# DerekGloudemans/3D-playground

Hardware: AMD Instinct MI355X
Metric: training images/sec at 1920x1080, ResNet-50 3D-RetinaNet (higher is better)
Workload: dtype f32; 1 GPU; resnet50 directional 3D-RetinaNet, 1920x1080 synthetic frames, batch 8 per GPU, 10 GT boxes/image, fp32, fwd+loss+bwd+clip+Adam (BASELINE configs[1]); global_batch=8, parallelism=dp1

## Files before the change

### 3d-playground_amd/csrc/conv_wino.hip

```cpp
#include "common.h"
#include "mfma_split.h"

__device__ __forceinline__ float4 f4(float s) { return make_float4(s, s, s, s); }
typedef float nt_f4 __attribute__((ext_vector_type(4)));
__device__ __forceinline__ float4 ld_stream(const float *p) {
    const nt_f4 v = __builtin_nontemporal_load(reinterpret_cast<const nt_f4 *>(p));
    return make_float4(v.x, v.y, v.z, v.w);
}
__device__ __forceinline__ void st_stream(float *p, float4 v) { *reinterpret_cast<float4 *>(p) = v; }
__device__ __forceinline__ float4 operator+(float4 a, float4 b) { return make_float4(a.x + b.x, a.y + b.y, a.z + b.z, a.w + b.w); }
__device__ __forceinline__ float4 operator-(float4 a, float4 b) { return make_float4(a.x - b.x, a.y - b.y, a.z - b.z, a.w - b.w); }
__device__ __forceinline__ float4 operator*(float s, float4 a) { return make_float4(s * a.x, s * a.y, s * a.z, s * a.w); }

__device__ __forceinline__ void bt6(const float4 d[6], float4 o[6]) {
    o[0] = 4.f * d[0] - 5.f * d[2] + d[4];
    o[1] = d[3] + d[4] - 4.f * (d[1] + d[2]);
    o[2] = 4.f * (d[1] - d[2]) - d[3] + d[4];
    o[3] = 2.f * (d[3] - d[1]) - d[2] + d[4];
    o[4] = 2.f * (d[1] - d[3]) - d[2] + d[4];
    o[5] = 4.f * d[1] - 5.f * d[3] + d[5];
}
__device__ __forceinline__ void at6(const float4 m[6], float4 o[4]) {
    const float4 s12 = m[1] + m[2], d12 = m[1] - m[2], s34 = m[3] + m[4], d34 = m[3] - m[4];
    o[0] = m[0] + s12 + s34;
// ... 16 lines not shown
    unsigned *amax[RN_MAX_GROUP];
};

#define WINO_GAIN_BT 7
#define WINO_GAIN_A 8
__device__ __forceinline__ void wino_tensor_word(const WinoTable &g, unsigned *tensor_amax, int gain) {
    if (tensor_amax == nullptr || blockIdx.x != 0 || threadIdx.x >= 64) return;
    int e = 0;
#pragma unroll
    for (int i = 0; i < RN_MAX_GROUP; ++i)
        if (i < g.n && g.amax[i] != nullptr) { const int ei = rn_amax_exp_all(g.amax[i], g.p[i].N); e = ei > e ? ei : e; }
    if (threadIdx.x == 0) atomicMax(tensor_amax, rn_amax_word_of_exp(e, gain));
}
__device__ __forceinline__ int wino_locate(const WinoTable &g, int64_t gt, int64_t &local) {
    int q = 0;
#pragma unroll
    for (int i = 0; i < RN_MAX_GROUP - 1; ++i) q += (i + 1 < g.n && gt >= g.tile_end[i]) ? 1 : 0;
    int64_t first = 0;
#pragma unroll
    for (int i = 1; i < RN_MAX_GROUP; ++i)
        if (q == i) first = g.tile_end[i - 1];
    local = gt - first;
    return q;
}

#define WINO_SELECT(q, g, pr, EXTRA)                          \
    WinoProblem pr = g.p[0];                                   \
    _Pragma("unroll") for (int i_ = 1; i_ < RN_MAX_GROUP; ++i_) \
        if (q == i_) { pr = g.p[i_]; EXTRA }

__global__ __launch_bounds__(256) void wino_in_kernel(const WinoTable g, float *__restrict__ V, int C, int64_t t0, int64_t Tpad,
                                                      unsigned *__restrict__ row_amax, unsigned *__restrict__ tensor_amax) {
    wino_tensor_word(g, tensor_amax, WINO_GAIN_BT);
    const int cq = C >> 2;
    const int64_t id = (int64_t)xcd_remap(blockIdx.x, gridDim.x) * 256 + threadIdx.x;
    const int64_t gt_raw = id / cq, t_last = g.tile_end[g.n - 1];
    const int64_t gt = gt_raw < t_last ? gt_raw : t_last - 1;
    const int c4 = (int)(id - gt_raw * cq) * 4;
    int64_t tile;
    const int q = wino_locate(g, gt, tile);
    const float *x = g.src[0];
    const unsigned *xw = g.amax[0];
    WINO_SELECT(q, g, pr, x = g.src[i_]; xw = g.amax[i_];)
    const int H = pr.H, W = pr.W, TW = pr.TW;
    const int n = (int)(tile / (pr.TH * TW));
    const int r = (int)(tile - (int64_t)n * pr.TH * TW);
    const int th = r / TW, tw = r - th * TW;
    const int h0 = 4 * th - 1, w0 = 4 * tw - 1;
    const float *xb = x + (int64_t)n * H * W * C + c4;
    if (row_amax != nullptr) {
        const int e_img = rn_amax_exp_lanes(xw != nullptr ? reinterpret_cast<const unsigned char *>(xw) + (int64_t)n * RN_AMAX_BYTES : nullptr);
        if (gt_raw < t_last && c4 == 0) row_amax[t0 + gt] = rn_amax_word_of_exp(e_img, WINO_GAIN_BT);
    }
    if (gt_raw >= t_last) return;
    float4 t[6][6];
#pragma unroll
    for (int j = 0; j < 6; ++j) {
        float4 d[6], o[6];
        const int w = w0 + j;
#pragma unroll
        for (int i = 0; i < 6; ++i) {
            const int h = h0 + i;
#ifdef RN_WINO_ABL
            const bool ok = (unsigned)h < (unsigned)H && (unsigned)w < (unsigned)W && i >= 1 && i <= 4 && j >= 1 && j <= 4;
#else
            const bool ok = (unsigned)h < (unsigned)H && (unsigned)w < (unsigned)W;
#endif
            d[i] = ok ? *reinterpret_cast<const float4 *>(xb + ((int64_t)h * W + w) * C) : f4(0.f);
        }
        bt6(d, o);
#pragma unroll
        for (int i = 0; i < 6; ++i) t[i][j] = o[i];
    }
    float *vb = V + (t0 + gt) * C + c4;
#pragma unroll
    for (int i = 0; i < 6; ++i) {
        float4 o[6];
        bt6(t[i], o);
#pragma unroll
        for (int j = 0; j < 6; ++j) st_stream(vb + (int64_t)(i * 6 + j) * Tpad * C, o[j]);
    }
}

template <bool PBITS, bool PADD, bool FLAGS = false>
__global__ __launch_bounds__(256, 2) void wino_out_kernel(const WinoTable g, const float *__restrict__ M, int Cout, int64_t t0,
                                                       int64_t Tpad, const float *__restrict__ scale,
                                                       const float *__restrict__ shift, int mask_mode, int act, int64_t y_bs,
                                                       const unsigned char *__restrict__ fin = nullptr,
                                                       unsigned char *__restrict__ fout = nullptr) {
    const int cq = Cout >> 2;
    const int64_t id = (int64_t)blockIdx.x * 256 + threadIdx.x;
    const int64_t gt = id / cq;
    float am = 0.f;
    unsigned *yam = nullptr;
    int n_img = 0;
    bool live = false;
    do {
    if (gt >= g.tile_end[g.n - 1]) break;
    live = true;
    const int c4 = (int)(id - gt * cq) * 4;
    int64_t tile;
    const int q = wino_locate(g, gt, tile);
    float *y = g.dst[0];
    const float *add = g.add[0], *mask = g.mask[0];
    unsigned *sign = g.sign[0];
    yam = g.amax[0];
    WINO_SELECT(q, g, pr, y = g.dst[i_]; add = g.add[i_]; mask = g.mask[i_]; sign = g.sign[i_]; yam = g.amax[i_];)
    n_img = (int)(tile / (pr.TH * pr.TW));
    const bool mbits = (mask_mode & RN_MASK_BITS) != 0;
    mask_mode &= 3;
    const int H = pr.H, W = pr.W, TW = pr.TW;
    const int n = (int)(tile / (pr.TH * TW));
    const int r = (int)(tile - (int64_t)n * pr.TH * TW);
    const int th = r / TW, tw = r - th * TW;
    const float *mb = M + (t0 + gt) * Cout + c4;
    float4 t[4][6];
    bool active = true;
    if constexpr (FLAGS) active = fin == nullptr || fin[t0 + gt] != 0;
    if (active) {
#pragma unroll
        for (int j = 0; j < 6; ++j) {
            float4 m[6], o[4];
#pragma unroll
            for (int i = 0; i < 6; ++i) m[i] = ld_stream(mb + (int64_t)(i * 6 + j) * Tpad * Cout);
            at6(m, o);
#pragma unroll
            for (int i = 0; i < 4; ++i) t[i][j] = o[i];
        }
    } else {
#pragma unroll
        for (int j = 0; j < 6; ++j)
#pragma unroll
            for (int i = 0; i < 4; ++i) t[i][j] = f4(0.f);
    }
    unsigned wake = 0u;
    float4 sc = f4(1.f), sh = f4(0.f);
    if (scale) sc = *reinterpret_cast<const float4 *>(scale + c4);
    if (shift) sh = *reinterpret_cast<const float4 *>(shift + c4);
    const int64_t ybs = y_bs ? y_bs : (int64_t)H * W * Cout;
#pragma unroll
    for (int i = 0; i < 4; ++i) {
        float4 o[4];
        at6(t[i], o);
        const int oh = 4 * th + i;
        if (oh >= H) break;
        unsigned mkw[4];
        float4 adv[4];
        if constexpr (PBITS || PADD) {
#pragma unroll
            for (int j = 0; j < 4; ++j) {
                const int owc = 4 * tw + j < W ? 4 * tw + j : W - 1;
                const int64_t off = (((int64_t)n * H + oh) * W + owc) * Cout + c4;
                if constexpr (PBITS) mkw[j] = reinterpret_cast<const unsigned *>(mask)[off >> 5] >> ((unsigned)off & 28u);
                if constexpr (PADD) adv[j] = *reinterpret_cast<const float4 *>(add + off);
            }
        }
#pragma unroll
        for (int j = 0; j < 4; ++j) {
            const int ow = 4 * tw + j;
            if (ow >= W) break;
            const int64_t off = (((int64_t)n * H + oh) * W + ow) * Cout + c4;
            const int64_t yoff = (int64_t)n * ybs + ((int64_t)oh * W + ow) * Cout + c4;
            float v[4] = {sc.x * o[j].x + sh.x, sc.y * o[j].y + sh.y, sc.z * o[j].z + sh.z, sc.w * o[j].w + sh.w};
            float mk[4] = {1.f, 1.f, 1.f, 1.f}, ad[4] = {0.f, 0.f, 0.f, 0.f};
            if constexpr (PBITS) {
                const unsigned nb = mkw[j];
                mk[0] = (nb & 1u) ? 1.f : 0.f; mk[1] = (nb & 2u) ? 1.f : 0.f; mk[2] = (nb & 4u) ? 1.f : 0.f; mk[3] = (nb & 8u) ? 1.f : 0.f;
            } else if (mask_mode != 0) { const float4 q4 = rn_mask_load4(mask, off, mbits); mk[0] = q4.x; mk[1] = q4.y; mk[2] = q4.z; mk[3] = q4.w; }
            if constexpr (PADD) { const float4 q4 = adv[j]; ad[0] = q4.x; ad[1] = q4.y; ad[2] = q4.z; ad[3] = q4.w; }
            else if (add) { const float4 q4 = *reinterpret_cast<const float4 *>(add + off); ad[0] = q4.x; ad[1] = q4.y; ad[2] = q4.z; ad[3] = q4.w; }
#pragma unroll
            for (int k = 0; k < 4; ++k) {
                float u = v[k];
                if (mask_mode == 1) u = mk[k] > 0.f ? u : 0.f;
                u += ad[k];
                if (act == 1) u = fmaxf(u, 0.f);
                else if (act == 2) u = 1.0f / (1.0f + expf(-u));
                if (mask_mode == 2) u = mk[k] > 0.f ? u : 0.f;
                v[k] = u;
            }
            *reinterpret_cast<float4 *>(y + yoff) = make_float4(v[0], v[1], v[2], v[3]);
            if (sign != nullptr) rn_sign_store(sign, off, v[0], v[1], v[2], v[3]);
            am = fmaxf(fmaxf(am, fmaxf(fabsf(v[0]), fabsf(v[1]))), fmaxf(fabsf(v[2]), fabsf(v[3])));
// ... 292 lines not shown
    int64_t end = 0;
    for (int i = 0; i < RN_MAX_GROUP; ++i) {
        const int k = i < g->n ? i : g->n - 1;
        if (g->N[k] <= 0 || g->H[k] <= 0 || g->W[k] <= 0) return RN_EINVAL;
        t.p[i].N = g->N[k]; t.p[i].H = g->H[k]; t.p[i].W = g->W[k];
        t.p[i].TH = (g->H[k] + 3) / 4; t.p[i].TW = (g->W[k] + 3) / 4;
        if (i < g->n) end += (int64_t)g->N[k] * t.p[i].TH * t.p[i].TW;
        t.tile_end[i] = end;
        t.src[i] = g->src[k]; t.dst[i] = g->dst[k]; t.add[i] = g->add[k]; t.mask[i] = g->mask[k];
        t.sign[i] = reinterpret_cast<unsigned *>(g->sign[k]);
        t.amax[i] = reinterpret_cast<unsigned *>(g->amax[k]);
    }
    return RN_OK;
}

extern "C" int rn_wino_input_group(const rn_wino_group *g, float *V, int C, int64_t tile_offset, int64_t Tpad, int dy_form,
                                   void *row_amax, void *tensor_amax, void *stream) {
    WinoTable t;
    const int rc = wino_table(g, t);
    if (rc) return rc;
    if (C <= 0 || (C & 3) || tile_offset < 0 || tile_offset + t.tile_end[t.n - 1] > Tpad) return RN_EINVAL;
    for (int i = 0; i < t.n; ++i)
        if (!t.src[i]) return RN_EINVAL;
    const dim3 grid(rn_blocks(t.tile_end[t.n - 1] * (C >> 2), 256));
    if (dy_form && row_amax != nullptr) return RN_EINVAL;
    if (dy_form) hipLaunchKernelGGL(wino_dy_kernel, grid, dim3(256), 0, (hipStream_t)stream, t, V, C, tile_offset, Tpad,
                                    reinterpret_cast<unsigned *>(tensor_amax));
    else hipLaunchKernelGGL(wino_in_kernel, grid, dim3(256), 0, (hipStream_t)stream, t, V, C, tile_offset, Tpad,
                            reinterpret_cast<unsigned *>(row_amax), reinterpret_cast<unsigned *>(tensor_amax));
    RN_LAUNCH_CHECK();
    return RN_OK;
}

extern "C" int rn_wino_input_both_group_flags(const rn_wino_group *g, float *V, float *Z, int C, int64_t tile_offset, int64_t Tpad,
                                              void *v_row_amax, void *z_tensor_amax, const void *flags, void *stream) {
    WinoTable t;
    const int rc = wino_table(g, t);
    if (rc) return rc;
    if (!V || !Z || C <= 0 || (C & 3) || tile_offset < 0 || tile_offset + t.tile_end[t.n - 1] > Tpad) return RN_EINVAL;
    if (flags != nullptr && (((uintptr_t)flags & 15) || (Tpad & 15))) return RN_EINVAL;
    for (int i = 0; i < t.n; ++i)
        if (!t.src[i]) return RN_EINVAL;
    const dim3 grid(rn_blocks(t.tile_end[t.n - 1] * (C >> 2), 256));
    if (flags != nullptr)
        hipLaunchKernelGGL(wino_in_both_kernel<true>, grid, dim3(256), 0, (hipStream_t)stream, t, V, Z, C, tile_offset, Tpad,
                           reinterpret_cast<unsigned *>(v_row_amax), reinterpret_cast<unsigned *>(z_tensor_amax),
                           reinterpret_cast<const unsigned char *>(flags));
    else
        hipLaunchKernelGGL(wino_in_both_kernel<false>, grid, dim3(256), 0, (hipStream_t)stream, t, V, Z, C, tile_offset, Tpad,
                           reinterpret_cast<unsigned *>(v_row_amax), reinterpret_cast<unsigned *>(z_tensor_amax),
                           (const unsigned char *)nullptr);
    RN_LAUNCH_CHECK();
    return RN_OK;
}
extern "C" int rn_tile_lists(const void *flags, int64_t Tpad, void *counts, void *tiles, void *units, void *blocks, void *stream) {
    if (!flags || !counts || !tiles || !units || !blocks || Tpad <= 0 || (Tpad & 255) || Tpad > 256 * 128) return RN_EINVAL;
    if (((uintptr_t)flags & 15) || (((uintptr_t)counts | (uintptr_t)tiles | (uintptr_t)units | (uintptr_t)blocks) & 3)) return RN_EINVAL;
    hipLaunchKernelGGL(tile_lists_kernel, dim3(1), dim3(256), 0, (hipStream_t)stream, reinterpret_cast<const unsigned char *>(flags), (int)Tpad,
                       reinterpret_cast<int *>(counts), reinterpret_cast<int *>(tiles), reinterpret_cast<int *>(units),
                       reinterpret_cast<int *>(blocks));
    RN_LAUNCH_CHECK();
    return RN_OK;
}

extern "C" int rn_wino_input_both_group_lists(const rn_wino_group *g, float *V, float *Z, int C, int64_t tile_offset, int64_t Tpad,
                                              void *v_row_amax, void *z_tensor_amax, const void *flags, const void *units,
                                              const void *n_units, void *stream) {
    WinoTable t;
    const int rc = wino_table(g, t);
    if (rc) return rc;
    if (!V || !Z || C <= 0 || (C & 3) || tile_offset < 0 || tile_offset + t.tile_end[t.n - 1] > Tpad) return RN_EINVAL;
    if (!flags || !units || !n_units || ((uintptr_t)flags & 15) || ((uintptr_t)units & 3) || (Tpad & 15)) return RN_EINVAL;
    for (int i = 0; i < t.n; ++i)
        if (!t.src[i]) return RN_EINVAL;
    const dim3 gl(rn_blocks(t.tile_end[t.n - 1] * (C >> 2), 256));
    hipLaunchKernelGGL((wino_in_both_kernel<true, true>), gl, dim3(256), 0, (hipStream_t)stream, t, V, Z, C, tile_offset, Tpad,
                       reinterpret_cast<unsigned *>(v_row_amax), reinterpret_cast<unsigned *>(z_tensor_amax),
                       reinterpret_cast<const unsigned char *>(flags), reinterpret_cast<const int *>(units),
                       reinterpret_cast<const int *>(n_units));
    RN_LAUNCH_CHECK();
    return RN_OK;
}

extern "C" int rn_wino_input_both_group(const rn_wino_group *g, float *V, float *Z, int C, int64_t tile_offset, int64_t Tpad,
                                        void *v_row_amax, void *z_tensor_amax, void *stream) {
    return rn_wino_input_both_group_flags(g, V, Z, C, tile_offset, Tpad, v_row_amax, z_tensor_amax, nullptr, stream);
}

extern "C" int rn_wino_output_group_flags(const rn_wino_group *g, const float *M, int Cout, int64_t tile_offset, int64_t Tpad,
                                          const float *scale, const float *shift, int mask_mode, int act, int64_t y_batch_stride,
                                          const void *flags_in, void *flags_out, void *stream) {
    WinoTable t;
    const int rc = wino_table(g, t);
    if (rc) return rc;
    if (Cout <= 0 || (Cout & 3) || tile_offset < 0 || tile_offset + t.tile_end[t.n - 1] > Tpad) return RN_EINVAL;
    if (mask_mode < 0 || (mask_mode & ~(3 | RN_MASK_BITS)) || (mask_mode & 3) == 3 || mask_mode == RN_MASK_BITS) return RN_EINVAL;
    if (act < 0 || act > 2 || y_batch_stride < 0 || (y_batch_stride & 3)) return RN_EINVAL;
    for (int i = 0; i < t.n; ++i) {
        if (!t.dst[i] || (mask_mode != 0) != (t.mask[i] != nullptr)) return RN_EINVAL;
        if (((mask_mode & RN_MASK_BITS) || t.sign[i]) && (Cout & 31)) return RN_EINVAL;
        if (y_batch_stride && y_batch_stride < (int64_t)t.p[i].H * t.p[i].W * Cout) return RN_EINVAL;
    }
    const bool pbits = (mask_mode & RN_MASK_BITS) != 0;
    bool padd = true;
    for (int i = 0; i < t.n; ++i) padd = padd && t.add[i] != nullptr;
    const dim3 grid(rn_blocks(t.tile_end[t.n - 1] * (Cout >> 2), 256));
    const unsigned char *fin = reinterpret_cast<const unsigned char *>(flags_in);
    unsigned char *fout = reinterpret_cast<unsigned char *>(flags_out);
#define RN_WINO_OUT(B, A, F) hipLaunchKernelGGL((wino_out_kernel<B, A, F>), grid, dim3(256), 0, (hipStream_t)stream, t, M, Cout, tile_offset, Tpad, \
                                                scale, shift, mask_mode, act, y_batch_stride, fin, fout)
    if (fin != nullptr || fout != nullptr) {
        if (pbits && padd) RN_WINO_OUT(true, true, true);
        else if (pbits) RN_WINO_OUT(true, false, true);
        else if (padd) RN_WINO_OUT(false, true, true);
        else RN_WINO_OUT(false, false, true);
    } else if (pbits && padd) RN_WINO_OUT(true, true, false);
    else if (pbits) RN_WINO_OUT(true, false, false);
    else if (padd) RN_WINO_OUT(false, true, false);
    else RN_WINO_OUT(false, false, false);
#undef RN_WINO_OUT
    RN_LAUNCH_CHECK();
    return RN_OK;
}
extern "C" int rn_wino_output_group(const rn_wino_group *g, const float *M, int Cout, int64_t tile_offset, int64_t Tpad,
                                    const float *scale, const float *shift, int mask_mode, int act, int64_t y_batch_stride,
                                    void *stream) {
    return rn_wino_output_group_flags(g, M, Cout, tile_offset, Tpad, scale, shift, mask_mode, act, y_batch_stride, nullptr, nullptr, stream);
}

static rn_wino_group wino_single(const float *src, float *dst, const float *add, const float *mask, int N, int H, int W) {
    rn_wino_group g = {};
    g.n = 1; g.N[0] = N; g.H[0] = H; g.W[0] = W; g.src[0] = src; g.dst[0] = dst; g.add[0] = add; g.mask[0] = mask;
    return g;
}
extern "C" int rn_wino_input(const float *x, float *V, int N, int H, int W, int C, int64_t tile_offset, int64_t Tpad,
                             void *stream) {
    const rn_wino_group g = wino_single(x, nullptr, nullptr, nullptr, N, H, W);
    return rn_wino_input_group(&g, V, C, tile_offset, Tpad, 0, nullptr, nullptr, stream);
}
extern "C" int rn_wino_dy(const float *dy, float *Z, int N, int H, int W, int C, int64_t tile_offset, int64_t Tpad, void *stream) {
    const rn_wino_group g = wino_single(dy, nullptr, nullptr, nullptr, N, H, W);
    return rn_wino_input_group(&g, Z, C, tile_offset, Tpad, 1, nullptr, nullptr, stream);
}
extern "C" int rn_wino_output(const float *M, float *y, int N, int H, int W, int Cout, int64_t tile_offset, int64_t Tpad,
                              const float *scale, const float *shift, const float *add, const float *mask, int mask_mode,
                              int act, int64_t y_batch_stride, void *stream) {
    const rn_wino_group g = wino_single(nullptr, y, add, mask, N, H, W);
    return rn_wino_output_group(&g, M, Cout, tile_offset, Tpad, scale, shift, mask_mode, act, y_batch_stride, stream);
}

extern "C" int rn_wino_weights(const float *w, float *U, int Cout, int Cin, int mode, const float *scale, void *stream) {
    if (Cout <= 0 || Cin <= 0 || mode < 0 || mode > 1) return RN_EINVAL;
    const int rows = mode == 0 ? Cout : Cin;
    const int Kpad = ((mode == 0 ? Cin : Cout) + 31) / 32 * 32;
    hipLaunchKernelGGL(wino_weight_kernel, dim3(rn_blocks((int64_t)rows * Kpad, 256)), dim3(256), 0, (hipStream_t)stream, w, U,
                       Cout, Cin, mode, scale, rows, Kpad);
    RN_LAUNCH_CHECK();
    return RN_OK;
}

extern "C" int rn_wino_dw(const float *dU, float *dw, int Cout, int Cin, void *stream) {
    if (Cout <= 0 || Cin <= 0) return RN_EINVAL;
    const int Ku = (Cin + 31) / 32 * 32, Kpad = (9 * Cin + 31) / 32 * 32;
    hipLaunchKernelGGL(wino_dw_kernel, dim3(rn_blocks((int64_t)Cout * Cin, 256)), dim3(256), 0, (hipStream_t)stream, dU, dw, Cout,
                       Cin, Ku, Kpad);
    RN_LAUNCH_CHECK();
    return RN_OK;
}
```

### 3d-playground_amd/csrc/focal_loss.hip

```cpp
#include <math.h>
#include <stdlib.h>

#include "common.h"

#ifndef FOCAL_NTHR
#define FOCAL_NTHR 256
#endif
#define NTHR FOCAL_NTHR
#define APT 4
#define TILE (NTHR * APT)
#define NWAVES (NTHR / 64)
#define UAPT 2
#define UNIT (64 * UAPT)
#define QCAP 256
#ifndef RN_FOCAL_WAVES_PER_SIMD
#define RN_FOCAL_WAVES_PER_SIMD 4
#endif
#define RN_FOCAL_WAVES_NOTE 4
#define RN_FOCAL_RESIDENT 768

static inline int focal_resident() {
    static const int v = [] { const char *e = getenv("RN_FOCAL_RESIDENT"); const int x = e ? atoi(e) : 0; return x >= 8 ? x : RN_FOCAL_RESIDENT; }();
    return v;
}
// ... 734 lines not shown
    const int units = (int)((A + UNIT - 1) / UNIT);
    const FocalWs ws = focal_ws(workspace, B);
    const dim3 grid((unsigned)(B * G)), block(NTHR);
    const float4 *anc = reinterpret_cast<const float4 *>(anchors);
    const int cq = C == 4 ? 1 : (C == 8 ? 2 : 0);
    const size_t raw_bytes = (size_t)(N > 0 ? N : 1) * (directional ? 27 : 5) * sizeof(float);
#define RN_FOCAL_FWD(DIR_, CQ_)                                                                                        \
    hipLaunchKernelGGL((focal_kernel<DIR_, false, CQ_>), grid, block, raw_bytes, s, cls, reg, anc, ann, A, C, N,        \
                       ws.partials, ws.stats, (float *)nullptr, (float *)nullptr, G, units, ws.counter, ws.terms, losses, \
                       (const float *)nullptr)
    if (directional) {
        if (cq == 2) RN_FOCAL_FWD(true, 2); else if (cq == 1) RN_FOCAL_FWD(true, 1); else RN_FOCAL_FWD(true, 0);
    } else {
        if (cq == 2) RN_FOCAL_FWD(false, 2); else if (cq == 1) RN_FOCAL_FWD(false, 1); else RN_FOCAL_FWD(false, 0);
    }
#undef RN_FOCAL_FWD
    RN_LAUNCH_CHECK();
    return RN_OK;
}

extern "C" int rn_focal_loss_bwd(const float *cls, const float *reg, const float *anchors, const float *ann, int B,
                                 int64_t A, int C, int N, int directional, const void *workspace,
                                 const float *grad_losses, float *dcls, float *dreg, void *stream) {
    const int rc = check_args(B, A, C, N);
    if (rc) return rc;
    hipStream_t s = (hipStream_t)stream;
    const int G = focal_groups(B, A);
    const int units = (int)((A + UNIT - 1) / UNIT);
    const FocalWs ws = focal_ws(const_cast<void *>(workspace), B);
    const dim3 grid((unsigned)(B * G)), block(NTHR);
    const float4 *anc = reinterpret_cast<const float4 *>(anchors);
    const int cq = C == 4 ? 1 : (C == 8 ? 2 : 0);
    const size_t raw_bytes = (size_t)(N > 0 ? N : 1) * (directional ? 27 : 5) * sizeof(float);
#define RN_FOCAL_BWD(DIR_, CQ_)                                                                                      \
    hipLaunchKernelGGL((focal_kernel<DIR_, true, CQ_>), grid, block, raw_bytes, s, cls, reg, anc, ann, A, C, N,       \
                       (float *)nullptr, ws.stats, dcls, dreg, G, units, (unsigned *)nullptr, (double *)nullptr,      \
                       (float *)nullptr, grad_losses)
    if (directional) {
        if (cq == 2) RN_FOCAL_BWD(true, 2); else if (cq == 1) RN_FOCAL_BWD(true, 1); else RN_FOCAL_BWD(true, 0);
    } else {
        if (cq == 2) RN_FOCAL_BWD(false, 2); else if (cq == 1) RN_FOCAL_BWD(false, 1); else RN_FOCAL_BWD(false, 0);
    }
#undef RN_FOCAL_BWD
    RN_LAUNCH_CHECK();
    return RN_OK;
}

template <bool DIR>
__global__ __launch_bounds__(NTHR) void assign_kernel(const float4 *__restrict__ anchors, const float *__restrict__ ann,
                                                      int64_t A, int N, float *__restrict__ iou_max,
                                                      int32_t *__restrict__ argmax, int32_t *__restrict__ state) {
    constexpr int COLS = DIR ? 27 : 5;
    __shared__ LabelLds L;
    const int j = blockIdx.y;
    load_labels<DIR>(ann + (int64_t)j * N * COLS, N, L);
    const int64_t ai = (int64_t)blockIdx.x * NTHR + threadIdx.x;
    if (ai >= A) return;
    float best = 0.f; int arg = -1; int st = 0;
    if (L.count > 0) {
        match_anchor(anchors[ai], L, best, arg);
        st = -1;
        if (best < 0.4f) st = 0;
        if (best >= 0.5f) st = 1;
    }
    iou_max[(int64_t)j * A + ai] = best;
    argmax[(int64_t)j * A + ai] = arg;
    state[(int64_t)j * A + ai] = st;
}

extern "C" int rn_assign(const float *anchors, const float *ann, int B, int64_t A, int N, int directional,
                         float *iou_max, int32_t *argmax, int32_t *state, void *stream) {
    const int rc = check_args(B, A, 1, N);
    if (rc) return rc;
    const dim3 grid((unsigned)((A + NTHR - 1) / NTHR), B), block(NTHR);
    const float4 *anc = reinterpret_cast<const float4 *>(anchors);
    if (directional)
        hipLaunchKernelGGL(assign_kernel<true>, grid, block, 0, (hipStream_t)stream, anc, ann, A, N, iou_max, argmax, state);
    else
        hipLaunchKernelGGL(assign_kernel<false>, grid, block, 0, (hipStream_t)stream, anc, ann, A, N, iou_max, argmax, state);
    RN_LAUNCH_CHECK();
    return RN_OK;
}

__global__ void pairwise_iou_kernel(const float4 *__restrict__ a, const float4 *__restrict__ b, float *__restrict__ out,
                                    int64_t A, int N) {
    const int64_t i = (int64_t)blockIdx.x * 256 + threadIdx.x;
    if (i >= A * N) return;
    const int64_t ai = i / N;
    const int n = (int)(i - ai * N);
    const float4 p = a[ai], q = b[n];
    const float area_b = (q.z - q.x) * (q.w - q.y);
    float iw = fminf(p.z, q.z) - fmaxf(p.x, q.x);
    float ih = fminf(p.w, q.w) - fmaxf(p.y, q.y);
    iw = fmaxf(iw, 0.f);
    ih = fmaxf(ih, 0.f);
    float ua = ((p.z - p.x) * (p.w - p.y) + area_b) - iw * ih;
    ua = fmaxf(ua, 1e-8f);
    out[i] = (iw * ih) / ua;
}

extern "C" int rn_pairwise_iou(const float *a, const float *b, float *iou, int64_t A, int N, void *stream) {
    if (A <= 0 || N <= 0) return RN_EINVAL;
    hipLaunchKernelGGL(pairwise_iou_kernel, dim3(rn_blocks(A * N, 256)), dim3(256), 0, (hipStream_t)stream,
                       reinterpret_cast<const float4 *>(a), reinterpret_cast<const float4 *>(b), iou, A, N);
    RN_LAUNCH_CHECK();
    return RN_OK;
}
```

### 3d-playground_amd/retinanet_mi355x/_hip.py

```python
import ctypes
import os

import torch

_HERE = os.path.dirname(os.path.abspath(__file__))
LIB_PATH = os.environ.get("RN_LIB_PATH") or os.path.join(_HERE, "lib", "libretinanet_mi355x.so")
_lib = None

c_i32, c_i64, c_f32, c_f64, c_vp = ctypes.c_int, ctypes.c_int64, ctypes.c_float, ctypes.c_double, ctypes.c_void_p

SIGNATURES = {
    "rn_version": (ctypes.c_char_p, []),
    "rn_check_device": (c_i32, []),
    "rn_get_fp32_mfma": (c_i32, []),
    "rn_set_fp32_mfma": (c_i32, [c_i32]),
    "rn_get_option": (c_i32, [c_i32]),
    "rn_set_option": (c_i32, [c_i32, c_i32]),
    "rn_fp32_split_min_k": (c_i32, []),
    "rn_split_weights": (c_i32, [c_vp, c_vp, c_i64, c_i32, c_vp]),
    "rn_split_weights_f16": (c_i32, [c_vp, c_vp, c_vp, c_i64, c_i32, c_vp]),
    "rn_amax": (c_i32, [c_vp, c_i64, c_i32, c_vp, c_vp]),
    "rn_stream_capture_id": (c_i32, [c_vp, ctypes.POINTER(ctypes.c_ulonglong)]),
    "rn_anchor_count": (c_i64, [c_i32, c_i32]),
    "rn_anchor_base_boxes": (None, [c_vp]),
    "rn_anchors_fwd": (c_i32, [c_vp, c_i32, c_i32, c_vp]),
    "rn_pairwise_iou": (c_i32, [c_vp, c_vp, c_vp, c_i64, c_i32, c_vp]),
    "rn_focal_workspace_bytes": (c_i64, [c_i32, c_i64]),
    "rn_focal_workspace_zero_bytes": (c_i64, [c_i32]),
    "rn_focal_loss_fwd": (c_i32, [c_vp, c_vp, c_vp, c_vp, c_i32, c_i64, c_i32, c_i32, c_i32, c_vp, c_vp, c_vp]),
    "rn_focal_loss_bwd": (c_i32, [c_vp, c_vp, c_vp, c_vp, c_i32, c_i64, c_i32, c_i32, c_i32, c_vp, c_vp, c_vp, c_vp, c_vp]),
    "rn_assign": (c_i32, [c_vp, c_vp, c_i32, c_i64, c_i32, c_i32, c_vp, c_vp, c_vp, c_vp]),
    "rn_decode_dir": (c_i32, [c_vp, c_vp, c_vp, c_i32, c_i64, c_vp]),
    "rn_decode_dir_select": (c_i32, [c_vp, c_vp, c_i64, c_vp, c_i64, c_vp, c_vp, c_i32, c_vp, c_vp, c_vp, c_vp]),
    "rn_decode_2d": (c_i32, [c_vp, c_vp, c_vp, c_i32, c_i64, c_i32, c_f32, c_f32, c_vp]),
    "rn_clip_boxes": (c_i32, [c_vp, c_i64, c_f32, c_f32, c_vp]),
    "rn_post_workspace_bytes": (c_i64, [c_i64, c_i64]),
    "rn_rowmax": (c_i32, [c_vp, c_i64, c_i32, c_vp, c_vp, c_vp]),
    "rn_threshold_select": (c_i32, [c_vp, c_i64, c_i64, c_f64, c_i32, c_f64, c_vp, c_vp, c_vp, c_vp]),
    "rn_nms": (c_i32, [c_vp, c_i64, c_i32, c_vp, c_i64, c_vp, c_vp, c_vp, c_i32, c_f32, c_vp, c_vp, c_vp, c_vp]),
    "rn_state_to_space": (c_i32, [c_vp, c_vp, c_i64, c_vp]),
    "rn_space_to_state": (c_i32, [c_vp, c_vp, c_i64, c_vp]),
    "rn_state_to_im": (c_i32, [c_vp, c_vp, c_vp, c_vp, c_vp, c_i64, c_vp]),
    "rn_space_to_im": (c_i32, [c_vp, c_vp, c_vp, c_vp, c_vp, c_i64, c_vp]),
    "rn_im_to_space": (c_i32, [c_vp, c_vp, c_vp, c_vp, c_vp, c_vp, c_i64, c_vp]),
    "rn_im_to_state": (c_i32, [c_vp, c_vp, c_vp, c_vp, c_vp, c_vp, c_i64, c_vp]),
    "rn_parse_workspace_bytes": (c_i64, [c_i64]),
    "rn_parse_detections": (c_i32, [c_vp, c_vp, c_vp, c_vp, c_i64, c_vp, c_vp, c_vp, c_vp, c_i32, c_vp, c_f32, c_f32, c_f32,
                                    c_i32, c_i32, c_vp, c_vp, c_vp, c_vp, c_vp, c_vp, c_vp]),
    "rn_md_iou": (c_i32, [c_vp, c_vp, c_vp, c_i64, c_vp]),
    "rn_crop_boxes": (c_i32, [c_vp, c_vp, c_i32, c_f64, c_vp, c_vp, c_vp]),
    "rn_roi_align": (c_i32, [c_vp, c_i32, c_i32, c_i32, c_i32, c_vp, c_i32, c_i32, c_i32, c_vp, c_i32, c_vp]),
    "rn_crop_select": (c_i32, [c_vp] * 9 + [c_i32] * 4 + [c_f64, c_i32, c_f32, c_vp, c_vp, c_vp, c_vp]),
    "rn_kf_view": (c_i32, [c_vp, c_vp, c_vp, c_vp, c_i32, c_i32, c_vp, c_i32, c_vp]),
    "rn_kf_predict": (c_i32, [c_vp, c_vp, c_vp, c_vp, c_vp, c_vp, c_vp, c_i32, c_f64, c_i32, c_vp]),
    "rn_kf_update": (c_i32, [c_vp, c_vp, c_vp, c_vp, c_vp, c_vp, c_vp, c_i32, c_vp]),
    "rn_track_cost": (c_i32, [c_vp, c_i64, c_vp, c_i64, c_i64, c_i64, c_vp, c_vp]),
    "rn_lsap_workspace_bytes": (c_i64, [c_i64, c_i64]),
    "rn_linear_sum_assignment": (c_i32, [c_vp, c_i64, c_i64, c_f64, c_vp, c_vp, c_vp, c_vp, c_vp]),
    "rn_ts_bias_workspace_bytes": (c_i64, [c_i64, c_i64]),
    "rn_estimate_ts_bias": (c_i32, [c_vp, c_i64, c_vp, c_i64, c_vp, c_vp, c_i64, c_i64, c_vp, c_vp, c_i32, c_f64, c_f64, c_f32,
                                    c_vp, c_i64, c_vp, c_vp, c_vp, c_vp]),
    "rn_track_crop_prior": (c_i32, [c_vp] * 7 + [c_i32, c_vp, c_vp, c_vp, c_i32, c_vp]),
    "rn_fit_nearest": (c_i32, [c_vp, c_vp, c_vp, c_i64, c_i64, c_vp, c_vp, c_vp, c_vp]),
    "rn_residual_moments": (c_i32, [c_vp, c_i64, c_i32, c_vp, c_i32, c_vp, c_vp, c_vp, c_vp]),
    "rn_eval_select": (c_i32, [c_vp, c_vp, c_vp, c_i64, c_i64, c_i64, c_f32, c_i32, c_i32, c_i64, c_i32, c_vp, c_i64, c_vp, c_vp, c_vp]),
    "rn_eval_match": (c_i32, [c_vp, c_i64, c_vp, c_i64, c_i32, c_vp, c_vp, c_i64, c_f64, c_vp, c_vp, c_vp, c_vp]),
    "rn_eval_ap_workspace_bytes": (c_i64, [c_i64]),
    "rn_eval_ap": (c_i32, [c_vp, c_i64, c_vp, c_vp, c_vp, c_i32, c_vp, c_vp, c_vp, c_vp]),
    "rn_eval_corners": (c_i32, [c_vp, c_i64, c_i64, c_i32, c_i64, c_vp, c_vp, c_i64, c_vp, c_vp]),
    "rn_eval_cuboid_overlap": (c_i32, [c_vp, c_i64, c_vp, c_i64, c_i32, c_vp, c_vp, c_vp, c_i64, c_i32, c_vp, c_vp, c_vp]),
    "rn_eval_cuboid_assign": (c_i32, [c_vp, c_i64, c_vp, c_i64, c_i32, c_vp, c_i64, c_vp, c_vp, c_vp, c_i32, c_vp, c_vp, c_vp,
                                      c_vp, c_vp]),
    "rn_eval_cuboid_errors": (c_i32, [c_vp, c_i64, c_vp, c_i64, c_i32, c_vp, c_vp, c_vp, c_i64, c_vp, c_vp, c_vp, c_vp, c_vp,
                                      c_vp]),
    "rn_frame_ingest": (c_i32, [c_vp, c_i32, c_i32, c_i32, c_i32] + [c_f32] * 6 + [c_i32, c_vp, c_vp]),
    "rn_frame_ingest_half": (c_i32, [c_vp, c_i32, c_i32, c_i32, c_i32] + [c_f32] * 6 + [c_i32, c_vp, c_vp, c_vp]),
    "rn_parse_frame_timestamps": (c_i32, [c_vp, c_i32, c_i32, c_i32, c_i64, c_i64, c_i32, c_vp, c_i32] + [c_vp] * 9),
    "rn_augment_workspace_bytes": (c_i64, [c_i32, c_i32, c_i32]),
    "rn_augment_frames": (c_i32, [c_vp, c_i32, c_i32, c_i32, c_vp, c_vp, c_vp, c_vp, ctypes.c_uint64] + [c_f32] * 6 + [c_vp, c_vp, c_vp]),
    "rn_augment_crops_workspace_bytes": (c_i64, [c_i32, c_i32, c_i32]),
    "rn_augment_crops": (c_i32, [c_vp, c_i32, c_i32, c_i32, c_vp, c_vp, c_vp, c_vp, c_vp, c_i32, c_i32, c_i32, c_vp, c_vp, ctypes.c_uint64]
                         + [c_f32] * 6 + [c_vp, c_vp, c_vp]),
    "rn_mot_prepare": (c_i32, [c_vp, c_vp, c_vp, c_i64, c_vp, c_i64] + [c_vp] * 7),
    "rn_mot_iou": (c_i32, [c_vp] * 5 + [c_i64, c_i64, c_vp, c_vp]),
    "rn_mot_assign": (c_i32, [c_vp] * 5 + [c_i64] * 4 + [c_vp] * 5),
    "rn_mot_frame_metrics": (c_i32, [c_vp] * 5 + [c_i64, c_i64, c_vp, c_vp, c_vp, c_f64] + [c_vp] * 19),
    "rn_mot_workspace_bytes": (c_i64, [c_i64, c_i64]),
    "rn_mot_reduce": (c_i32, [c_i64, c_i64] + [c_vp] * 16 + [c_i64, c_i64, c_vp, c_vp, c_vp]),
    "rn_mot_assoc_workspace_bytes": (c_i64, [c_i64, c_i64]),
    "rn_mot_id_counts": (c_i32, [c_vp] * 5 + [c_i64] * 6 + [c_vp, c_vp, c_i64, c_i64, c_f64] + [c_vp] * 5),
    "rn_mot_id_assign": (c_i32, [c_vp, c_i64, c_i64, c_vp, c_vp, c_vp, c_vp]),
    "rn_mot_hota_align": (c_i32, [c_vp] * 5 + [c_i64] * 6 + [c_vp] * 5 + [c_i64] * 3 + [c_vp] * 5),
    "rn_mot_hota_assign": (c_i32, [c_vp] * 5 + [c_i64] * 6 + [c_vp, c_vp, c_i64, c_i64] + [c_vp] * 11),
    "rn_mot_hota_reduce": (c_i32, [c_vp] * 4 + [c_i64] * 6 + [c_vp] * 9 + [c_i64, c_i64, c_vp, c_vp, c_vp]),
    "rn_vanishing_points": (c_i32, [c_vp, c_i64, c_vp, c_i64, c_vp, c_vp, c_vp, c_vp]),
    "rn_hg_reproj_error": (c_i32, [c_vp, c_vp, c_vp, c_vp, c_vp, c_i64, c_i64, c_vp, c_vp]),
    "rn_hg_scale_z": (c_i32, [c_vp, c_vp, c_vp, c_vp, c_i64, c_f64, c_f64, c_i32, c_vp, c_vp, c_vp, c_vp]),
    "rn_fit_homography": (c_i32, [c_vp, c_vp, c_i64, c_vp, c_i64, c_i32, c_vp, c_vp, c_vp]),
    "rn_reinterp_mate": (c_i32, [c_vp, c_vp, c_i64, c_i64, c_vp, c_vp, c_vp]),
    "rn_reinterp_offsets": (c_i32, [c_vp, c_vp, c_i64, c_i64, c_vp, c_i64] + [c_vp] * 5),
    "rn_reinterp_rows": (c_i32, [c_vp] * 7 + [c_i64] * 4 + [c_vp] * 5),
    "rn_track_rows": (c_i32, [c_vp] * 5 + [c_i64, c_i64] + [c_vp] * 7),
    "rn_render_edges": (c_i32, [c_vp, c_vp, c_i64, c_i32, c_i32, c_vp, c_i32, c_i32, c_i32, c_vp]),
    "rn_render_rects": (c_i32, [c_vp, c_i64, c_vp, c_i64, c_vp, c_i32, c_i32, c_i32, c_vp]),
    "rn_render_text": (c_i32, [c_vp, c_i64, c_vp, c_i64, c_vp, c_vp, c_i64, c_vp, c_i32, c_i32, c_i32, c_vp]),
    "rn_render_compose": (c_i32, [c_vp] + [c_f32] * 6 + [c_vp, c_i32, c_vp, c_i32, c_i32, c_i32, c_i32, c_vp]),
    "rn_replay_boxes": (c_i32, [c_vp, c_i64, c_vp, c_vp, c_vp, c_i32, c_vp, c_vp, c_vp, c_vp, c_vp]),
    "rn_replay_compose": (c_i32, [c_vp, c_i32, c_vp, c_vp] + [c_i32] * 6 + [c_vp]),
    "rn_frame_absdiff": (c_i32, [c_vp, c_vp] + [c_i32] * 6 + [c_vp, c_vp, c_vp]),
    "rn_running_frame": (c_i32, [c_vp, c_vp, c_i64, c_i32, c_vp]),
    "rn_label_pair_samples": (c_i32, [c_vp, c_vp, c_i64, c_i32, c_i64, c_i32, c_i32, c_i32, c_vp, c_vp, c_vp, c_vp]),
    "rn_label_outliers": (c_i32, [c_vp, c_vp, c_vp, c_i64, c_i64, c_i64, c_i64, c_vp, c_vp, c_vp]),
    "rn_label_interpolate_workspace_bytes": (c_i64, [c_i64, c_i64]),
    "rn_label_interpolate": (c_i32, [c_vp] * 4 + [c_i64] * 3 + [c_i32, c_i64] + [c_vp] * 7),
    "rn_label_rebase": (c_i32, [c_vp, c_vp, c_i64] + [c_vp] * 4 + [c_i32, c_vp, c_i32, c_i32] + [c_vp] * 5),
    "rn_label_offset_y": (c_i32, [c_vp] * 4 + [c_i64, c_i32, c_vp, c_vp]),
    "rn_label_crop_windows": (c_i32, [c_vp, c_vp, c_i64, c_vp, c_vp, c_i32, c_f32, c_f32, c_f32] + [c_vp] * 6),
    "rn_label_best_anchor": (c_i32, [c_vp, c_vp, c_vp, c_i64, c_i32, c_i32, c_f32] + [c_vp] * 5),
    "rn_label_fit_box2d": (c_i32, [c_vp] * 5 + [c_i64, c_vp, c_vp, c_i32, c_vp, c_i32, c_i32] + [c_vp] * 5),
    "rn_spline_fit_workspace_bytes": (c_i64, [c_i64, c_i32]),
    "rn_label_box_weights": (c_i32, [c_vp, c_vp, c_i64, c_vp, c_vp, c_i32, c_vp, c_vp, c_vp]),
    "rn_spline_fit": (c_i32, [c_vp, c_i64, c_vp, c_i64, c_vp, c_vp, c_vp, c_i64, c_vp, c_i64, c_i32] + [c_vp] * 7),
    "rn_spline_select": (c_i32, [c_vp, c_i64] + [c_vp] * 4 + [c_i64, c_i64, c_i64, c_i32] + [c_vp] * 4 + [c_i32] + [c_vp] * 7),
    "rn_spline_eval": (c_i32, [c_vp, c_vp, c_vp, c_i64, c_i32, c_vp, c_vp, c_i64, c_vp, c_vp]),
    "rn_label_ts_shift": (c_i32, [c_vp, c_vp, c_vp, c_i64, c_i32, c_vp, c_vp, c_vp, c_i64, c_i64, c_vp, c_vp, c_vp, c_i32, c_i32,
                                  c_i32] + [c_vp] * 5),
    "rn_label_series_workspace_bytes": (c_i64, [c_i64]),
    "rn_label_series": (c_i32, [c_vp, c_vp, c_i64, c_i32, c_i64, c_i32, c_f64, c_f64, c_i32] + [c_vp] * 8),
    "rn_label_group_rmse": (c_i32, [c_vp, c_vp, c_i64, c_i64] + [c_vp] * 5),
    "rn_stitch_endpoints": (c_i32, [c_vp, c_vp, c_vp, c_i64, c_i64, c_i32, c_vp, c_vp, c_vp]),
    "rn_stitch_costs": (c_i32, [c_vp, c_i64] + [c_f64] * 7 + [c_vp, c_vp]),
    "rn_stitch_candidates": (c_i32, [c_vp, c_i64] + [c_f64] * 7 + [c_vp] * 4),
    "rn_stitch_compact": (c_i32, [c_vp, c_i64] + [c_f64] * 7 + [c_vp, c_vp, c_i64, c_vp, c_vp, c_vp]),
    "rn_stitch_assign_workspace_bytes": (c_i64, [c_i64]),
    "rn_stitch_assign": (c_i32, [c_vp, c_i64] + [c_f64] * 7 + [c_vp, c_vp, c_vp, c_i64] + [c_vp] * 6),
    "rn_stitch_chains": (c_i32, [c_vp, c_vp, c_i64] + [c_vp] * 6),
    "rn_stitch_fill_count": (c_i32, [c_vp, c_vp, c_i64, c_f64] + [c_vp] * 4),
    "rn_stitch_fill_rows": (c_i32, [c_vp, c_vp, c_vp, c_i64, c_i64, c_f64] + [c_vp] * 6),
    "rn_smooth_filter": (c_i32, [c_vp] * 5 + [c_f64, c_f64, c_i64, c_i64] + [c_vp] * 5),
    "rn_smooth_rts": (c_i32, [c_vp] * 5 + [c_f64, c_i64, c_i64] + [c_vp] * 4),
    "rn_traffic_lanes": (c_i32, [c_vp] * 4 + [c_i32, c_vp, c_i32, c_i64, c_i64] + [c_vp] * 4),
    "rn_traffic_cells": (c_i32, [c_vp] * 4 + [c_i32, c_vp, c_i32, c_i64, c_i64, c_f64, c_f64, c_i64, c_f64, c_f64, c_i64, c_f64] + [c_vp] * 6),
    "rn_traffic_leaders": (c_i32, [c_vp] * 6 + [c_i64] * 4 + [c_vp] * 8),
}

class ConvDesc(ctypes.Structure):
    _fields_ = [("N", c_i32), ("Hi", c_i32), ("Wi", c_i32), ("Cin", c_i32),
                ("Ho", c_i32), ("Wo", c_i32), ("Cout", c_i32),
                ("kh", c_i32), ("kw", c_i32),
                ("a", c_i32), ("b", c_i32), ("p", c_i32), ("p_w", c_i32), ("div_shift", c_i32),
                ("act", c_i32), ("add_mode", c_i32), ("Ha", c_i32), ("Wa", c_i32),
                ("mask_mode", c_i32), ("in_relu", c_i32),
                ("os", c_i32), ("oo_h", c_i32), ("oo_w", c_i32), ("Hy", c_i32), ("Wy", c_i32),
                ("add2_mode", c_i32), ("Ha2", c_i32), ("Wa2", c_i32), ("add2_batch_stride", c_i64),
                ("x_batch_stride", c_i64), ("y_batch_stride", c_i64), ("add_batch_stride", c_i64),
                ("w_batch_stride", c_i64), ("w_format", c_i32), ("sign_out", c_vp),
                ("x_amax", c_vp), ("y_amax", c_vp), ("w_unscale", c_vp), ("x_amax_img_stride", c_i32), ("x_amax_row_stride", c_i32),
                ("row_active", c_vp), ("row_list", c_vp), ("row_list_n", c_vp), ("row_list_grid", c_i32)]


RN_MAX_GROUP = 5


class ConvGroup(ctypes.Structure):
    _fields_ = [("n", c_i32), ("tile_end", c_i32 * RN_MAX_GROUP), ("d", ConvDesc * RN_MAX_GROUP),
                ("x", c_vp * RN_MAX_GROUP), ("y", c_vp * RN_MAX_GROUP), ("add", c_vp * RN_MAX_GROUP),
                ("mask", c_vp * RN_MAX_GROUP)]


class PrepJob(ctypes.Structure):
    _fields_ = [("kind", c_i32)] + [(n, c_i32) for n in ("Cout", "Cin", "kh", "kw", "kw_pad", "c_pad", "mode", "r0", "nr", "s0",
                                                          "ns", "rows", "Kpad")] + \
               [("eps", c_f32), ("src", c_vp), ("dst", c_vp), ("scale", c_vp), ("gamma", c_vp), ("beta", c_vp), ("mean", c_vp),
                ("var", c_vp), ("bn_scale", c_vp), ("bn_shift", c_vp), ("bn_rstd", c_vp)]


class UnpackJob(ctypes.Structure):
    _fields_ = [("dw", c_vp), ("w_packed", c_vp), ("dweight", c_vp)] + \
               [(n, c_i32) for n in ("Cout", "Cin", "kh", "kw", "kw_pad", "c_pad", "Kpad")] + \
               [("scale", c_vp), ("mean", c_vp), ("rstd", c_vp), ("colsum", c_vp), ("dgamma", c_vp), ("dbeta", c_vp)]


class WinoGroup(ctypes.Structure):
    _fields_ = [("n", c_i32), ("N", c_i32 * RN_MAX_GROUP), ("H", c_i32 * RN_MAX_GROUP), ("W", c_i32 * RN_MAX_GROUP),
                ("src", c_vp * RN_MAX_GROUP), ("dst", c_vp * RN_MAX_GROUP), ("add", c_vp * RN_MAX_GROUP),
                ("mask", c_vp * RN_MAX_GROUP), ("sign", c_vp * RN_MAX_GROUP), ("amax", c_vp * RN_MAX_GROUP)]


SIGNATURES.update({
    "rn_unpack_batched": (c_i32, [c_vp, c_vp, c_i32, c_vp]),
    "rn_prep_batched": (c_i32, [c_vp, c_vp, c_i32, c_vp]),
    "rn_wino_input_group": (c_i32, [ctypes.POINTER(WinoGroup), c_vp, c_i32, c_i64, c_i64, c_i32, c_vp, c_vp, c_vp]),
    "rn_wino_input_both_group": (c_i32, [ctypes.POINTER(WinoGroup), c_vp, c_vp, c_i32, c_i64, c_i64, c_vp, c_vp, c_vp]),
    "rn_wino_input_both_group_flags": (c_i32, [ctypes.POINTER(WinoGroup), c_vp, c_vp, c_i32, c_i64, c_i64, c_vp, c_vp, c_vp, c_vp]),
    "rn_tile_lists": (c_i32, [c_vp, c_i64, c_vp, c_vp, c_vp, c_vp, c_vp]),
    "rn_wino_input_both_group_lists": (c_i32, [ctypes.POINTER(WinoGroup), c_vp, c_vp, c_i32, c_i64, c_i64, c_vp, c_vp, c_vp, c_vp, c_vp, c_vp]),
    "rn_wino_output_group_flags": (c_i32, [ctypes.POINTER(WinoGroup), c_vp, c_i32, c_i64, c_i64, c_vp, c_vp, c_i32, c_i32, c_i64, c_vp, c_vp, c_vp]),
    "rn_wino_output_group": (c_i32, [ctypes.POINTER(WinoGroup), c_vp, c_i32, c_i64, c_i64, c_vp, c_vp, c_i32, c_i32, c_i64, c_vp]),
    "rn_conv_igemm_grouped": (c_i32, [ctypes.POINTER(ConvGroup), c_vp, c_vp, c_vp, c_vp]),
    "rn_conv_igemm": (c_i32, [ctypes.POINTER(ConvDesc), c_vp, c_vp, c_vp, c_vp, c_vp, c_vp, c_vp, c_vp, c_vp]),
    "rn_conv_splitk_workspace_bytes": (c_i64, [ctypes.POINTER(ConvDesc)]),
    "rn_conv_igemm_wants_f16": (c_i32, [ctypes.POINTER(ConvDesc)]),
    "rn_conv_igemm_splitk": (c_i32, [ctypes.POINTER(ConvDesc)] + [c_vp] * 10),
    "rn_conv_wgrad": (c_i32, [c_vp, c_i32, c_vp, c_vp, c_vp] + [c_i32] * 12 + [c_vp]),
    "rn_pack_weights": (c_i32, [c_vp, c_vp] + [c_i32] * 7 + [c_vp] + [c_i32] * 4 + [c_vp]),
    "rn_unpack_wgrad": (c_i32, [c_vp, c_vp, c_vp] + [c_i32] * 6 + [c_vp] * 7),
    "rn_bn_fold": (c_i32, [c_vp, c_vp, c_vp, c_vp, c_f32, c_i32, c_vp, c_vp, c_vp, c_vp]),
    "rn_nchw_to_nhwc4": (c_i32, [c_vp, c_vp, c_i32, c_i32, c_i32, c_vp, c_vp]),
    "rn_maxpool_fwd": (c_i32, [c_vp, c_vp, c_vp] + [c_i32] * 6 + [c_vp]),
    "rn_maxpool_bwd": (c_i32, [c_vp, c_vp, c_vp, c_vp] + [c_i32] * 7 + [c_vp, c_vp]),
    "rn_colsum": (c_i32, [c_vp, c_i64, c_i32, c_i32, c_vp, c_i32, c_vp, c_vp]),
    "rn_colsum_workspace_bytes": (c_i64, [c_i64, c_i32]),
    "rn_upsample_add_bwd": (c_i32, [c_vp, c_vp] + [c_i32] * 6 + [c_vp, c_vp]),
    "rn_relu_mask": (c_i32, [c_vp, c_vp, c_i64, c_vp]),
    "rn_sigmoid_bwd_pad": (c_i32, [c_vp, c_vp, c_vp, c_i32, c_i64, c_i32, c_i32, c_i64, c_vp, c_vp]),
    "rn_sigmoid_bwd_pad_flags": (c_i32, [c_vp, c_vp, c_vp, c_i32, c_i32, c_i32, c_i32, c_i32, c_i64, c_vp, c_vp, c_vp]),
    "rn_add_inplace": (c_i32, [c_vp, c_vp, c_i64, c_i64, c_vp, c_vp]),
    "rn_wino_input": (c_i32, [c_vp, c_vp, c_i32, c_i32, c_i32, c_i32, c_i64, c_i64, c_vp]),
    "rn_wino_output": (c_i32, [c_vp, c_vp, c_i32, c_i32, c_i32, c_i32, c_i64, c_i64, c_vp, c_vp, c_vp, c_vp, c_i32, c_i32, c_i64, c_vp]),
    "rn_wino_weights": (c_i32, [c_vp, c_vp, c_i32, c_i32, c_i32, c_vp, c_vp]),
    "rn_wino_dy": (c_i32, [c_vp, c_vp, c_i32, c_i32, c_i32, c_i32, c_i64, c_i64, c_vp]),
    "rn_wino_dw": (c_i32, [c_vp, c_vp, c_i32, c_i32, c_vp]),
    "rn_conv_wgrad_batched": (c_i32, [c_vp, c_i32, c_vp, c_vp, c_vp, c_i32, c_i64, c_i64, c_i64, c_i32] + [c_i32] * 12 + [c_vp, c_i32, c_vp, c_i32, c_vp]),
    "rn_conv_wgrad_batched_det": (c_i32, [c_vp, c_i32, c_vp, c_vp, c_vp, c_i32, c_i64, c_i64, c_i64, c_i32] + [c_i32] * 12 + [c_vp, c_i32, c_vp, c_i32, c_vp, c_i64, c_vp]),
    "rn_conv_wgrad_batched_flags": (c_i32, [c_vp, c_i32, c_vp, c_vp, c_vp, c_i32, c_i64, c_i64, c_i64, c_i32] + [c_i32] * 12 + [c_vp, c_i32, c_vp, c_i32, c_vp, c_vp, c_i64, c_vp]),
    "rn_conv_wgrad_det_workspace_bytes": (c_i64, [c_i32, c_i32, c_i64] + [c_i32] * 9),
    "rn_conv_wgrad_plan": (c_i32, [c_i32, c_i32, c_i64, c_i64, c_i64, c_i32] + [c_i32] * 12 + [c_i32, c_i32, c_i32, c_vp]),
    "rn_conv_bwd_1x1": (c_i32, [c_vp] * 8 + [c_i32] + [c_vp] * 5 + [c_i32] * 6 + [c_vp]),
    "rn_f32_to_bf16": (c_i32, [c_vp, c_vp, c_i64, c_vp]),
    "rn_bf16_to_f32": (c_i32, [c_vp, c_vp, c_i64, c_vp]),
    "rn_conv_igemm_bf16": (c_i32, [ctypes.POINTER(ConvDesc), c_vp, c_vp, c_vp, c_i32, c_vp, c_vp, c_vp, c_vp, c_vp]),
    "rn_conv_igemm_bf16_grouped": (c_i32, [ctypes.POINTER(ConvGroup), c_vp, c_i32, c_vp, c_vp, c_vp]),
    "rn_conv_igemm_bf16_tile_rows": (c_i32, [ctypes.POINTER(ConvGroup), c_i32]),
    "rn_maxpool_fwd_fp8out": (c_i32, [c_vp, c_vp] + [c_i32] * 6 + [c_f32, c_vp]),
    "rn_conv_igemm_fp8_tile_rows": (c_i32, [ctypes.POINTER(ConvGroup), c_i32]),
    "rn_conv_igemm_fp8_tile": (c_i32, [ctypes.POINTER(ConvDesc), c_i32]),
    "rn_conv_igemm_bf16_tile": (c_i32, [ctypes.POINTER(ConvDesc), c_i32]),
    "rn_fp8_quantize": (c_i32, [c_vp, c_vp, c_i64, c_f32, c_vp]),
    "rn_fp8_dequantize": (c_i32, [c_vp, c_vp, c_i64, c_f32, c_vp]),
    "rn_fp8_to_bf16": (c_i32, [c_vp, c_vp, c_i64, c_f32, c_vp]),
    "rn_bf16_to_fp8": (c_i32, [c_vp, c_vp, c_i64, c_f32, c_vp]),
    "rn_fp8_quantize_rows": (c_i32, [c_vp, c_vp, c_vp, c_i64, c_i32, c_vp]),
    "rn_conv_igemm_fp8": (c_i32, [ctypes.POINTER(ConvDesc), c_vp, c_vp, c_vp, c_i32, c_vp, c_vp, c_vp, c_f32, c_f32, c_vp]),
    "rn_conv_igemm_fp8_grouped": (c_i32, [ctypes.POINTER(ConvGroup), c_vp, c_i32, c_vp, c_vp, c_f32, c_f32, c_vp]),
    "rn_conv_wgrad_bf16": (c_i32, [c_vp, c_i32, c_vp, c_vp, c_vp] + [c_i32] * 11 + [c_vp]),
    "rn_conv_wgrad_bf16_grouped": (c_i32, [c_i32, ctypes.POINTER(c_vp), c_i32, ctypes.POINTER(c_vp), c_vp, c_vp, c_i32,
                                           ctypes.POINTER(c_i32), ctypes.POINTER(c_i32)] + [c_i32] * 6 + [c_vp]),
    "rn_maxpool_fwd_bf16out": (c_i32, [c_vp, c_vp, c_vp] + [c_i32] * 6 + [c_vp]),
    "rn_maxpool_bwd_bf16in": (c_i32, [c_vp, c_vp, c_vp, c_vp] + [c_i32] * 7 + [c_vp]),
    "rn_upsample_add_bwd_bf16": (c_i32, [c_vp, c_vp] + [c_i32] * 6 + [c_vp]),
    "rn_sigmoid_bwd_pad_bf16": (c_i32, [c_vp, c_vp, c_vp, c_i32, c_i64, c_i32, c_i32, c_i64, c_vp]),
    "rn_relu_bf16": (c_i32, [c_vp, c_vp, c_i64, c_vp]),
    "rn_opt_workspace_bytes": (c_i64, [c_i32]),
    "rn_opt_clip_adam": (c_i32, [c_vp, c_vp, c_i32, c_f32, c_f32, c_f32, c_f32, c_f32, c_i32, c_i32, c_vp, c_vp, c_vp]),
    "rn_opt_clip_adam_dev": (c_i32, [c_vp, c_vp, c_i32, c_f32, c_f32, c_f32, c_f32, c_f32, c_vp, c_i32, c_vp, c_vp, c_vp]),
    "rn_opt_clip_adam_hp": (c_i32, [c_vp, c_vp, c_i32, c_vp, c_vp, c_i32, c_vp, c_vp, c_vp]),
})


RN_ERRORS = {10001: "RN_EINVAL (bad size / unsupported shape)",
             10002: "RN_ETOOMANY (more than RN_MAX_GT=256 label rows per image)"}


def load():
    global _lib
    if _lib is None:
        if not os.path.exists(LIB_PATH):
            raise RuntimeError(
                "libretinanet_mi355x.so is missing (%s): build it with `python -c 'import __graft_entry__ as g; "
                "g.build()'` or `make -C 3d-playground_amd/csrc`.  There is no CPU fallback." % LIB_PATH)
        lib = ctypes.CDLL(LIB_PATH)
        for name, (res, args) in SIGNATURES.items():
            fn = getattr(lib, name)
            fn.restype = res
            fn.argtypes = args
        _lib = lib
    return _lib

# ... 34 lines not shown
```

### 3d-playground_amd/retinanet_mi355x/conv.py

```python
import ctypes
import os

import torch

from . import _hip, prof

ConvDesc = _hip.ConvDesc

ACT_NONE, ACT_RELU, ACT_SIGMOID = 0, 1, 2


def kpad(kh, kw, c):
    return (kh * kw * c + 31) // 32 * 32


def out_size(n, k, stride, pad):
    return (n + 2 * pad - k) // stride + 1


def pack_weights(weight, mode=0, scale=None, kw_pad=None, c_pad=None, taps=None, presplit=True):
    lib = _hip.load()
    w = _hip.f32c(weight.detach())
    _hip.need_gpu(w, scale)
    cout, cin, kh, kw = w.shape
# ... 286 lines not shown
                return 1
            ws = torch.empty(nb, dtype=torch.uint8, device=dev)
        return lib.rn_conv_wgrad_batched_flags(dy_ptr, ldy, x_ptr, dw_ptr, cs_ptr, nbatch, dy_bs, x_bs, dw_bs, cs_batch, *geom, *am,
                                               flags.data_ptr(), _hip.ptr(ws), nb, _hip.stream())
    if not lib.rn_get_option(OPT_DETERMINISTIC):
        return lib.rn_conv_wgrad_batched(dy_ptr, ldy, x_ptr, dw_ptr, cs_ptr, nbatch, dy_bs, x_bs, dw_bs, cs_batch, *geom, *am, _hip.stream())
    N, Hi, Wi, Cin, Ho, Wo, Cout, kh, kw = geom[:9]
    nb = lib.rn_conv_wgrad_det_workspace_bytes(ldy, nbatch, dw_bs, N, Hi, Wi, Cin, Ho, Wo, Cout, kh, kw)
    if nb < 0:
        return 1
    ws = torch.empty(nb, dtype=torch.uint8, device=dev)
    return lib.rn_conv_wgrad_batched_det(dy_ptr, ldy, x_ptr, dw_ptr, cs_ptr, nbatch, dy_bs, x_bs, dw_bs, cs_batch, *geom, *am,
                                         ws.data_ptr(), nb, _hip.stream())


WGRAD_PLAN_FIELDS = ("shape", "tiles", "splits", "per_split", "xcd_map", "grid", "kernel", "arith")


def wgrad_plan(ldy, nbatch, dy_bs, x_bs, dw_bs, cs_batch, geom, have_amax=False, have_flags=False, det=None):
    out = (ctypes.c_int32 * 8)()
    det = get_option(OPT_DETERMINISTIC) if det is None else det
    rc = _hip.load().rn_conv_wgrad_plan(ldy, nbatch, dy_bs, x_bs, dw_bs, cs_batch, *geom, int(have_amax), int(have_flags), int(det), out)
    return dict(zip(WGRAD_PLAN_FIELDS, out)) if rc == 0 else None


def wino_weights(weight, mode=0, scale=None):
    lib = _hip.load()
    w = _hip.f32c(weight.detach())
    _hip.need_gpu(w, scale)
    cout, cin, kh, kw = w.shape
    assert kh == 3 and kw == 3
    rows, k = (cout, cin) if mode == 0 else (cin, cout)
    U = torch.empty((36, rows, (k + 31) // 32 * 32), dtype=torch.float32, device=w.device)
    _hip.check(lib.rn_wino_weights(w.data_ptr(), U.data_ptr(), cout, cin, mode, _hip.ptr(scale), _hip.stream()),
               "rn_wino_weights")
    return _maybe_split(U, rows=rows, cin=U.shape[2], taps=1)


_WINO_WS = {}
_WINO_ODD_PLANES = os.environ.get("RN_WINO_ODD_PLANES", "1") != "0"


def wino_tpad(T):
    n = (T + 255) // 256
    if _WINO_ODD_PLANES and n % 2 == 0:
        n += 1
    return n * 256


def _wino_group(xs, srcs=None, dsts=None, adds=None, masks=None, mask_bits=False, signs=None, amaxs=None):
    g = _hip.WinoGroup()
    g.n = len(xs)
    for i, x in enumerate(xs):
        g.N[i], g.H[i], g.W[i] = x.shape[0], x.shape[1], x.shape[2]
        g.src[i] = None if srcs is None else srcs[i].data_ptr()
        g.dst[i] = None if dsts is None else dsts[i].data_ptr()
        g.add[i] = None if adds is None or adds[i] is None else adds[i].data_ptr()
        if masks is None or masks[i] is None:
            g.mask[i] = None
        else:
            g.mask[i] = masks[i]._rn_sign.data_ptr() if mask_bits else masks[i].data_ptr()
        g.sign[i] = None if signs is None or signs[i] is None else signs[i].data_ptr()
        g.amax[i] = None if amaxs is None or amaxs[i] is None else amaxs[i].data_ptr()
    return g


def _wino_transform_in(xs, V, C, Tpad, dy_form, want_rows=False, want_tensor=False):
    lib = _hip.load()
    off = 0
    am = want_amax() and (want_rows or want_tensor)
    rows = torch.zeros(Tpad, dtype=torch.int32, device=V.device) if am and want_rows else None
    tword = amax_single(V.device) if am and want_tensor else None
    for k in range(0, len(xs), _hip.RN_MAX_GROUP):
        part = xs[k:k + _hip.RN_MAX_GROUP]
        t = sum(x.shape[0] * ((x.shape[1] + 3) // 4) * ((x.shape[2] + 3) // 4) for x in part)
        g = _wino_group(part, srcs=part, amaxs=[amax_words(x) for x in part] if am else None)
        nb = 4.0 * (sum(x.numel() for x in part) + 36 * t * C)
        _hip.check(prof.timed("wino_input", nb, lambda: lib.rn_wino_input_group(
            ctypes.byref(g), V.data_ptr(), C, off, Tpad, dy_form, _hip.ptr(rows), _hip.ptr(tword), _hip.stream())), "rn_wino_input_group")
        off += t
    return rows, tword


def _wino_workspace(device, floats_v, floats_m):
    key = (device, torch.cuda.current_stream(device).cuda_stream)
    ws = _WINO_WS.get(key)
    if ws is None or ws[0].numel() < floats_v or ws[1].numel() < floats_m:
        ws = (torch.empty(max(floats_v, ws[0].numel() if ws else 0), dtype=torch.float32, device=device),
              torch.empty(max(floats_m, ws[1].numel() if ws else 0), dtype=torch.float32, device=device))
        _WINO_WS[key] = ws
    return ws


def tile_flags(device, T):
    return torch.zeros(wino_tpad(T), dtype=torch.uint8, device=device)


class TileLists:
    __slots__ = ("flags", "buf", "counts", "tiles", "units", "blocks", "grid")

    def lengths(self):
        return tuple(int(v) for v in self.counts[:3].tolist())


def tile_lists_numel(Tpad):
    return 4 + Tpad + Tpad // 16 + Tpad // 128


def tile_lists(flags, Tpad=None, buf=None, grid=0):
    lib = _hip.load()
    Tpad = flags.numel() if Tpad is None else Tpad
    assert flags.dtype == torch.uint8 and flags.numel() >= Tpad and Tpad % 256 == 0
    n = tile_lists_numel(Tpad)
    if buf is None:
        buf = torch.empty(n, dtype=torch.int32, device=flags.device)
    assert buf.dtype == torch.int32 and buf.numel() >= n and buf.is_contiguous()
    tl = TileLists()
    tl.flags, tl.buf, tl.grid = flags, buf, int(grid)
    nb, nu = Tpad // 128, Tpad // 16
    tl.counts, tl.blocks, tl.units, tl.tiles = buf[:4], buf[4:4 + nb], buf[4 + nb:4 + nb + nu], buf[4 + nb + nu:n]
    _hip.check(lib.rn_tile_lists(flags.data_ptr(), Tpad, tl.counts.data_ptr(), tl.tiles.data_ptr(), tl.units.data_ptr(),
                                 tl.blocks.data_ptr(), _hip.stream()), "rn_tile_lists")
    return tl


def wino_flags_ok(T, C, cout):
    lib = _hip.load()
    return bool(get_fp32_mfma() != "native" and lib.rn_get_option(OPT_WGRAD_ONCE) and C > 64 and cout > 64 and T < 32000)


def wino_conv_group(xs, U, outs=None, scale=None, shift=None, act=ACT_NONE, adds=None, masks=None, mask_mode=2,
                    flops=0.0, keep_v=False, y_batch_stride=0, V_in=None, V_ready=None, sign=False, flags_out=None):
    lib = _hip.load()
    dev = xs[0].device
    C = xs[0].shape[3]
    cout = U.shape[1]
    tiles = [x.shape[0] * ((x.shape[1] + 3) // 4) * ((x.shape[2] + 3) // 4) for x in xs]
    T = sum(tiles)
    Tpad = wino_tpad(T)
    V, M = _wino_workspace(dev, 0 if keep_v else 36 * Tpad * C, 36 * Tpad * cout)
    shapes = tuple(tuple(x.shape) for x in xs)
    reuse = keep_v and V_in is not None and V_in[1] == shapes and V_in[0].numel() == 36 * Tpad * C
    ready = not keep_v and isinstance(V_ready, tuple) and V_ready[1] == shapes and V_ready[0].numel() >= 36 * Tpad * C
    if ready:
        V, reuse = V_ready[0], True
    elif reuse:
        V = V_in[0]
    elif keep_v:
        V = torch.empty(36 * Tpad * C, dtype=torch.float32, device=dev)
    assert all(x.is_contiguous() for x in xs)
    v_am = (None, None)
    if reuse:
        src = V_ready if ready else V_in
        v_am = src[2] if len(src) > 2 and src[2] is not None else (None, None)
    else:
        v_am = _wino_transform_in(xs, V, C, Tpad, 0, want_rows=True, want_tensor=keep_v)
    flags = V_ready[3] if ready and len(V_ready) > 3 else None
    lists = V_ready[4] if ready and len(V_ready) > 4 else None
    if flags_out is not None:
        assert flags_out.dtype == torch.uint8 and flags_out.numel() >= Tpad and len(xs) <= _hip.RN_MAX_GROUP
    Vv = V[:36 * Tpad * C].view(36, 1, Tpad, C)
    Mv = M[:36 * Tpad * cout].view(36, 1, Tpad, cout)
    Uv = _carry_split(U, U.view(36 * cout, U.shape[2]))
    if want_amax() and v_am[0] is None:
        Uv = U.view(36 * cout, U.shape[2])
    conv_igemm(Vv, Uv, Mv, (1, Tpad, cout, 1, 1, 1, 1, 0, 0), flops=2.0 * 36 * T * cout * C, w_batch_stride=cout * U.shape[2],
               x_amax=v_am[0], x_amax_rows=True, row_active=flags, row_list=lists)
    if outs is None:
        outs = [torch.empty((x.shape[0], x.shape[1], x.shape[2], cout), dtype=torch.float32, device=dev) for x in xs]
    off = 0
    for k in range(0, len(xs), _hip.RN_MAX_GROUP):
        sl = slice(k, k + _hip.RN_MAX_GROUP)
        part, t = xs[sl], sum(tiles[sl])
        pa = None if adds is None else adds[sl]
        pm = None if masks is None else masks[sl]
        has_mask = pm is not None and pm[0] is not None
        mbits = has_mask and BITMASKS and all(getattr(m, "_rn_sign", None) is not None for m in pm)
        for o in outs[sl]:
            amax_drop(o)
        signs = [_sign_words(o, sign and not y_batch_stride) for o in outs[sl]]
        yams = [amax_slot(dev, o.shape[0]) for o in outs[sl]] if want_amax() and not y_batch_stride else None
        g = _wino_group(part, dsts=outs[sl], adds=pa, masks=pm, mask_bits=mbits, signs=signs, amaxs=yams)
        nops = 1 + (pa is not None and pa[0] is not None) + (1.0 / 32 if mbits else 1.0) * has_mask + (1.0 / 32 if signs[0] is not None else 0.0)
        nb = 4.0 * (36 * t * cout + nops * sum(x.shape[0] * x.shape[1] * x.shape[2] for x in part) * cout)
        mm = (mask_mode | (MASK_BITS if mbits else 0)) if has_mask else 0
        if flags is not None or flags_out is not None:
            _hip.check(prof.timed("wino_output", nb, lambda: lib.rn_wino_output_group_flags(
                ctypes.byref(g), M.data_ptr(), cout, off, Tpad, _hip.ptr(scale), _hip.ptr(shift), mm,
                act, y_batch_stride, _hip.ptr(flags), _hip.ptr(flags_out), _hip.stream())), "rn_wino_output_group_flags")
        else:
            _hip.check(prof.timed("wino_output", nb, lambda: lib.rn_wino_output_group(
                ctypes.byref(g), M.data_ptr(), cout, off, Tpad, _hip.ptr(scale), _hip.ptr(shift), mm,
                act, y_batch_stride, _hip.stream())), "rn_wino_output_group")
        if yams is not None:
            for o, w_ in zip(outs[sl], yams):
                amax_attach(o, w_)
        off += t
    return (outs, (V, tuple(tuple(x.shape) for x in xs), v_am)) if keep_v else outs


_WINO_Z = {}
SIDE_HELD = {}


def side_release(side=None):
    if side is None:
        SIDE_HELD.clear()
    else:
        SIDE_HELD.pop(side.cuda_stream, None)


def _wino_z_buffer(device, floats):
    cur = torch.cuda.current_stream(device)
    st = _WINO_Z.setdefault((device, cur.cuda_stream), {"bufs": [None, None], "ev": [None, None], "i": 0})
    k = st["i"]
    st["i"] ^= 1
    if st["bufs"][k] is None or st["bufs"][k].numel() < floats:
        st["bufs"][k] = torch.empty(floats, dtype=torch.float32, device=device)
    if st["ev"][k] is not None:
        cur.wait_event(st["ev"][k])
    return st, k


def wino_wgrad_group(gs, xs, dw, colsum, flops=0.0, V=None, dU=None, fuse_dgrad_input=False, side=None, flags=None, lists=None):
    lib = _hip.load()
    dev = xs[0].device
    C, cout = xs[0].shape[3], gs[0].shape[3]
    zst = None
    tiles = [x.shape[0] * ((x.shape[1] + 3) // 4) * ((x.shape[2] + 3) // 4) for x in xs]
    T = sum(tiles)
    Tpad = wino_tpad(T)
    have_v = V is not None and V[1] == tuple(tuple(x.shape) for x in xs) and V[0].numel() == 36 * Tpad * C
    v_tw = V[2][1] if have_v and len(V) > 2 and V[2] is not None else None
    V = V[0] if have_v else None
    Vw, Z = _wino_workspace(dev, 0 if have_v else 36 * Tpad * C, 36 * Tpad * cout)
    if not have_v:
        V = Vw
    assert all(g.shape[:3] == x.shape[:3] and g.is_contiguous() and x.is_contiguous() for g, x in zip(gs, xs))
    if not have_v:
        v_tw = _wino_transform_in(xs, V, C, Tpad, 0, want_tensor=True)[1]
    v_dy, z_tw = None, None
    if fuse_dgrad_input and have_v and len(gs) <= _hip.RN_MAX_GROUP:
        Vd, Z = _wino_workspace(dev, 36 * Tpad * cout, 36 * Tpad * cout)
        if side is not None:
            zst, zk = _wino_z_buffer(dev, 36 * Tpad * cout)
            Z = zst["bufs"][zk]
        am_on = want_amax()
        g = _wino_group(gs, srcs=gs, amaxs=[amax_words(t) for t in gs] if am_on else None)
        vd_rows = torch.zeros(Tpad, dtype=torch.int32, device=dev) if am_on else None
        z_tw = amax_single(dev) if am_on else None
        nb = 4.0 * (sum(t.numel() for t in gs) + 2 * 36 * T * cout)
        if flags is not None and not wino_flags_ok(T, C, cout):
            flags = None
        if flags is not None:
            assert flags.dtype == torch.uint8 and flags.numel() >= Tpad
        if flags is None or lists is None or lists is False:
            lists = None
        elif not isinstance(lists, TileLists):
            lists = tile_lists(flags, Tpad, buf=None if lists is True else lists)
        if lists is not None:
            assert lists.flags.data_ptr() == flags.data_ptr()
            _hip.check(prof.timed("wino_input", nb, lambda: lib.rn_wino_input_both_group_lists(
                ctypes.byref(g), Vd.data_ptr(), Z.data_ptr(), cout, 0, Tpad, _hip.ptr(vd_rows), _hip.ptr(z_tw), flags.data_ptr(),
                lists.units.data_ptr(), lists.counts.data_ptr() + 4, _hip.stream())), "rn_wino_input_both_group_lists")
        else:
            _hip.check(prof.timed("wino_input", nb, lambda: lib.rn_wino_input_both_group_flags(
                ctypes.byref(g), Vd.data_ptr(), Z.data_ptr(), cout, 0, Tpad, _hip.ptr(vd_rows), _hip.ptr(z_tw), _hip.ptr(flags),
                _hip.stream())), "rn_wino_input_both_group_flags")
        v_dy = (Vd, tuple(tuple(t.shape) for t in gs), (vd_rows, None)) + ((flags,) if flags is not None else ()) \
# ... 603 lines not shown
```

### 3d-playground_amd/retinanet_mi355x/engine.py

```python
import os

import torch

from . import _hip, arch, conv as cv, ops, prof


FUSE_DY = os.environ.get("RN_WINO_FUSE_DY", "1") != "0"
SPARSE_REG = os.environ.get("RN_SPARSE_REG", "1") != "0"
SPARSE_REG_LISTS = os.environ.get("RN_SPARSE_REG_LISTS", "1") != "0"
GROUPED_WGRAD_BF16 = os.environ.get("RN_GROUPED_WGRAD_BF16", "1") != "0"
S2_SHORTCUT_COMPACT = os.environ.get("RN_S2_SHORTCUT_COMPACT", "1") != "0"
STEM_BF16_PRODUCTS = os.environ.get("RN_STEM_BF16_PRODUCTS", "1") != "0"


def _qscale(t):
    return getattr(t, "_rn_scale", None) or getattr(t, "_rn_qscale", None)


def _as_fp8(t):
    if t is None or t.dtype == torch.uint8:
        return t
    q = getattr(t, "_rn_q8", None)
    if q is None:
        sc = _qscale(t)
        assert sc, "a tensor entering an fp8 layer needs its calibrated scale (Layer.fwd tags its outputs)"
        q = t._rn_q8 = cv.fp8_quantize(t, sc) if t.dtype == torch.float32 else cv.bf16_to_fp8(t, sc)
    return q


def _as_f32(t):
    if t is None or t.dtype == torch.float32:
        return t
    y = cv.fp8_dequantize(t) if t.dtype == torch.uint8 else cv.to_f32(t)
    y._rn_qscale = _qscale(t)
    return y


def _as_bf16(t):
    if t is None or t.dtype == torch.bfloat16:
        return t
    y = cv.fp8_to_bf16(t) if t.dtype == torch.uint8 else cv.to_bf16(t)
    y._rn_qscale = _qscale(t)
    return y


_AS = {"fp8": _as_fp8, "bf16": _as_bf16, "fp32": _as_f32}


class Layer:

    def __init__(self, spec, kw_pad=None, cin_pad=None, bf16=False, fp8=False):
        self.spec = spec
        self.bf16 = bf16
        self.fp8 = fp8
        self.out_scale = 1.0
        self.calib = None
        self.kw_pad = spec.k if kw_pad is None else kw_pad
        self.cin_pad = spec.cin if cin_pad is None else cin_pad
        self.cout_pad = (spec.cout + 31) // 32 * 32 if spec.cout % (8 if bf16 else 4) else spec.cout
        self.wino_ok = spec.k == 3 and spec.stride == 1 and spec.pad == 1 and spec.cin % 4 == 0 and spec.cout % 4 == 0
        self.wino_layer = self.wino_ok and min(spec.cin, spec.cout) >= 64 and max(spec.cin, spec.cout) >= 128 and not bf16
        self.wino_active = False
        self.sign = False
        self.keep_v = True
        self._cache = None
        self.reset()

    def reset(self):
        self.wf = self.wd = self.scale = self.shift = self.rstd = self.mean = None
        self.dw = self.cs = None
        self.uf = self.ud = None
        self.wf16 = self.wd16 = None
        self.saved_v = None
        self.dy_v = None

    def prepare(self, P, cache):
        s = self.spec
        self._cache = cache
        w = P[s.name + ".weight"]
        self.weight = w
        self.wf = cache.get(("wf", s.name), w, lambda: cv.pack_weights(w, 0, kw_pad=self.kw_pad, c_pad=self.cin_pad))
        if s.bn:
            g, b = P[s.bn + ".weight"], P[s.bn + ".bias"]
            self.mean = P[s.bn + ".running_mean"]
            self.scale, self.shift, self.rstd = cache.get(
                ("bn", s.bn), (g, b), lambda: cv.bn_fold(g, b, self.mean, P[s.bn + ".running_var"], arch.BN_EPS))
        else:
            self.scale = self.rstd = self.mean = None
            self.shift = P[s.name + ".bias"].detach() if s.bias else None
        self.wd = None
        self.dw = self.cs = None
        self.uf = self.ud = None
# ... 27 lines not shown
            self._fp8_scales = {}

    def wino_weights(self, mode):
        if mode == 0:
            if self.uf is None:
                self.uf = self._cache.get(("uf", self.spec.name), self.weight, lambda: cv.wino_weights(self.weight, 0)) \
                    if self._cache is not None else cv.wino_weights(self.weight, 0)
            return self.uf
        if self.ud is None:
            self.ud = cv.wino_weights(self.weight, 1, scale=self.scale)
        return self.ud

    def dgrad_weights16(self):
        if self.wd16 is None:
            wd = self.dgrad_weights()
            self.wd16 = [cv.to_bf16(t) for t in wd] if isinstance(wd, list) else cv.to_bf16(wd)
        return self.wd16

    def dgrad_weights(self):
        if self.wd is None:
            s = self.spec
            if s.stride == 2 and s.k > 1:
                self.wd = [cv.pack_weights(self.weight, 1, scale=self.scale, c_pad=self.cout_pad, taps=c[2])
                           for c in cv.s2_classes(s.k, s.pad)]
            else:
                self.wd = cv.pack_weights(self.weight, 1, scale=self.scale, c_pad=self.cout_pad)
        return self.wd

    def fwd(self, x, act=cv.ACT_NONE, add=None, add_mode=0, add_hw=(0, 0), out=None, y_batch_stride=None, in_relu=False, sign=None):
        s = self.spec
        sign = (self.sign and act == cv.ACT_RELU) if sign is None else (sign and self.sign)
        N, Hi, Wi, _ = x.shape
        Ho, Wo = cv.out_size(Hi, s.k, s.stride, s.pad), cv.out_size(Wi, s.k, s.stride, s.pad)
        mode = self.mode()
        if self.fp8:
            x, add = _AS[mode](x), _AS[mode](add)
        if mode == "fp8":
            assert not in_relu, "fp8: the caller applies the input ReLU"
            return self._fwd_fp8(x, (Ho, Wo), act, add, add_mode, add_hw, out, y_batch_stride)
        if mode == "bf16":
            assert not in_relu, "bf16: the caller applies the input ReLU (cv.relu_bf16)"
            if out is None:
                out = torch.empty((N, Ho, Wo, s.cout), dtype=torch.bfloat16, device=x.device)
            cv.conv_igemm_bf16(x, self.wf16, out, (Ho, Wo, s.cout, s.k, self.kw_pad, s.stride, 1, -s.pad, 0),
                               scale=self.scale, shift=self.shift, add=add, add_mode=add_mode, add_hw=add_hw, act=act,
                               y_batch_stride=y_batch_stride, flops=self.flops(N, Ho, Wo), sign=sign)
            out._rn_qscale = self.out_scale
            return out
        if self.wino_active and out is None and add is None and not in_relu and y_batch_stride is None \
                and act in (cv.ACT_NONE, cv.ACT_RELU) and x.is_contiguous():
            r = cv.wino_conv_group([x], self.wino_weights(0), scale=self.scale, shift=self.shift, act=act, keep_v=self.keep_v, sign=sign)
            ys, self.saved_v = r if self.keep_v else (r, None)
            return ys[0]
        if out is None:
            out = torch.empty((N, Ho, Wo, s.cout), dtype=torch.float32, device=x.device)
        cv.conv_igemm(x, self.wf, out, (Ho, Wo, s.cout, s.k, self.kw_pad, s.stride, 1, -s.pad, 0), scale=self.scale,
                      shift=self.shift, add=add, add_mode=add_mode, add_hw=add_hw, act=act,
                      y_batch_stride=y_batch_stride, in_relu=in_relu, flops=self.flops(N, Ho, Wo), sign=sign,
                      bf16_products=getattr(self, "bf16_products", False))
        self._tap(out if y_batch_stride is None else None)
        out._rn_qscale = self.out_scale
        return out

    def mode(self):
        return getattr(self, "fwd_mode", None) or ("fp8" if self.fp8 else ("bf16" if self.bf16 else "fp32"))

    def _tap(self, out):
        if self.calib is not None and out is not None:
            self.calib[self.spec.name] = max(self.calib.get(self.spec.name, 0.0), float(out.abs().max()))

    def _fwd_fp8(self, x, out_hw, act, add, add_mode, add_hw, out, y_batch_stride):
        s = self.spec
        Ho, Wo = out_hw
        sx = float(x._rn_scale)
        scale = self._fp8_scales.get(sx)
        if scale is None:
            scale = self._fp8_scales[sx] = (self.wscale * sx).contiguous()
        if out is None:
            out = torch.empty((x.shape[0], Ho, Wo, s.cout), dtype=torch.uint8, device=x.device)
        return cv.conv_igemm_fp8(x, self.wq, out, (Ho, Wo, s.cout, s.k, self.kw_pad, s.stride, 1, -s.pad, 0), scale, shift=self.shift,
                                 add=add, add_mode=add_mode, add_hw=add_hw, act=act, y_batch_stride=y_batch_stride,
                                 out_scale=self.out_scale, flops=self.flops(x.shape[0], Ho, Wo))

    def fwd_group(self, xs, act=cv.ACT_NONE, outs=None, y_batch_stride=None, wino=False, shared_v=None):
        s = self.spec
        mode = self.mode()
        if self.fp8:
            xs = [_AS[mode](x) for x in xs]
        if mode == "fp8":
            scales = {float(x._rn_scale) for x in xs}
            if len(scales) > 1 or len(xs) > _hip.RN_MAX_GROUP:
                return [self._fwd_fp8(x, (x.shape[1], x.shape[2]), act, None, 0, (0, 0), None if outs is None else outs[i], y_batch_stride)
                        for i, x in enumerate(xs)]
            sx = scales.pop()
            scale = self._fp8_scales.get(sx)
            if scale is None:
                scale = self._fp8_scales[sx] = (self.wscale * sx).contiguous()
            probs, ys, fl = [], [], 0.0
            for i, x in enumerate(xs):
                N, Hi, Wi, _ = x.shape
                y = outs[i] if outs is not None else torch.empty((N, Hi, Wi, s.cout), dtype=torch.uint8, device=x.device)
                ys.append(y)
                fl += self.flops(N, Hi, Wi)
                probs.append({"x": x, "y": y, "geom": (Hi, Wi, s.cout, s.k, self.kw_pad, 1, 1, -s.pad, 0), "y_batch_stride": y_batch_stride})
            cv.conv_igemm_fp8_grouped(probs, self.wq, scale, shift=self.shift, act=act, out_scale=self.out_scale, flops=fl)
            return ys
        if mode == "bf16":
            probs, ys, fl = [], [], 0.0
            for i, x in enumerate(xs):
                N, Hi, Wi, _ = x.shape
                y = outs[i] if outs is not None else torch.empty((N, Hi, Wi, s.cout), dtype=torch.bfloat16, device=x.device)
                ys.append(y)
                fl += self.flops(N, Hi, Wi)
                probs.append({"x": x, "y": y, "geom": (Hi, Wi, s.cout, s.k, self.kw_pad, 1, 1, -s.pad, 0),
                              "y_batch_stride": y_batch_stride, "sign": self.sign and act == cv.ACT_RELU})
            cv.conv_igemm_bf16_grouped(probs, self.wf16, scale=self.scale, shift=self.shift, act=act, flops=fl)
            for y in ys:
                y._rn_qscale = self.out_scale
            return ys
        if (wino or self.wino_active) and self.wino_ok and (outs is None or y_batch_stride is not None):
            fl = sum(self.flops(x.shape[0], x.shape[1], x.shape[2]) for x in xs)
            r = cv.wino_conv_group(xs, self.wino_weights(0), outs=outs, scale=self.scale, shift=self.shift, act=act, flops=fl,
                                   keep_v=self.keep_v, y_batch_stride=y_batch_stride or 0, V_in=shared_v if self.keep_v else None,
                                   sign=self.sign and act == cv.ACT_RELU)
            ys, self.saved_v = r if self.keep_v else (r, None)
            return ys
        probs, ys, fl = [], [], 0.0
        for i, x in enumerate(xs):
            N, Hi, Wi, _ = x.shape
            Ho, Wo = cv.out_size(Hi, s.k, s.stride, s.pad), cv.out_size(Wi, s.k, s.stride, s.pad)
            y = outs[i] if outs is not None else torch.empty((N, Ho, Wo, s.cout), dtype=torch.float32, device=x.device)
            ys.append(y)
            fl += self.flops(N, Ho, Wo)
            probs.append({"x": x, "y": y, "geom": (Ho, Wo, s.cout, s.k, self.kw_pad, s.stride, 1, -s.pad, 0),
                          "y_batch_stride": y_batch_stride, "sign": self.sign and act == cv.ACT_RELU})
        cv.conv_igemm_grouped(probs, self.wf, scale=self.scale, shift=self.shift, act=act, flops=fl)
        if outs is None:
            for y in ys:
                self._tap(y)
                y._rn_qscale = self.out_scale
        return ys

    def bwd_data_group(self, gs, in_hws, adds=None, masks=None, wino=False, flags_out=None):
        s = self.spec
        assert s.stride == 1
        self.flags_out_done = False
        if self.bf16:
            probs, outs, fl = [], [], 0.0
            for i, g in enumerate(gs):
                Hi, Wi = in_hws[i]
                dx = torch.empty((g.shape[0], Hi, Wi, s.cin), dtype=torch.bfloat16, device=g.device)
                outs.append(dx)
                fl += self.flops(g.shape[0], g.shape[1], g.shape[2])
                probs.append({"x": g, "y": dx, "geom": (Hi, Wi, s.cin, s.k, s.k, 1, -1, s.pad, 0),
                              "add": None if adds is None else adds[i], "mask": None if masks is None else masks[i]})
            cv.conv_igemm_bf16_grouped(probs, self.dgrad_weights16(), flops=fl)
            return outs
        if (wino or self.wino_active) and self.wino_ok and all(g.shape[3] == s.cout for g in gs):
            fl = sum(self.flops(g.shape[0], g.shape[1], g.shape[2]) for g in gs)
            ready, self.dy_v = getattr(self, "dy_v", None), None
            self.flags_out_done = flags_out is not None
            return cv.wino_conv_group(gs, self.wino_weights(1), adds=adds, masks=masks, mask_mode=2, flops=fl, V_ready=ready,
                                      flags_out=flags_out)
        probs, outs, fl = [], [], 0.0
        for i, g in enumerate(gs):
            N = g.shape[0]
            Hi, Wi = in_hws[i]
            dx = torch.empty((N, Hi, Wi, s.cin), dtype=torch.float32, device=g.device)
            outs.append(dx)
            fl += self.flops(N, g.shape[1], g.shape[2])
            probs.append({"x": g, "y": dx, "geom": (Hi, Wi, s.cin, s.k, s.k, 1, -1, s.pad, 0),
                          "add": None if adds is None else adds[i], "mask": None if masks is None else masks[i]})
        cv.conv_igemm_grouped(probs, self.dgrad_weights(), flops=fl)
        return outs

    def flops(self, N, Ho, Wo):
        s = self.spec
        return 2.0 * N * Ho * Wo * s.cout * s.cin * s.k * s.k

    def bwd_params(self, g, x, in_relu=False, side=None):
        s = self.spec
        if self.dw is None:
            self.dw = torch.zeros_like(self.wf)
            self.cs = torch.zeros(s.cout, dtype=torch.float32, device=g.device)
        if self.bf16:
            assert not in_relu
            cv.wgrad_bf16(g, x, self.dw, s.cout, s.k, s.stride, s.pad, flops=self.flops(g.shape[0], g.shape[1], g.shape[2]),
                          colsum=self.cs)
            return
        if self.wino_active and not in_relu and g.shape[3] == s.cout and g.is_contiguous() and x.is_contiguous():
            du, self.du = getattr(self, "du", None), None
            self.dy_v = cv.wino_wgrad_group([g], [x], self.dw, self.cs, V=self.saved_v, dU=du, fuse_dgrad_input=FUSE_DY, side=side)
            self.saved_v = None
            return
        cv.wgrad(g, x, self.dw, s.cout, s.k, s.stride, s.pad, kw_pad=self.kw_pad, in_relu=in_relu,
                 flops=self.flops(g.shape[0], g.shape[1], g.shape[2]), colsum=self.cs)

    def bwd_params_group(self, gs, xs, wino=False, side=None, flags=None, lists=None):
        s = self.spec
        if (wino or self.wino_active) and self.wino_ok and all(g.shape[3] == s.cout and g.is_contiguous() for g in gs):
            if self.dw is None:
                self.dw = torch.zeros_like(self.wf)
                self.cs = torch.zeros(s.cout, dtype=torch.float32, device=gs[0].device)
            fl = sum(self.flops(g.shape[0], g.shape[1], g.shape[2]) for g in gs)
            du, self.du = getattr(self, "du", None), None
            self.dy_v = cv.wino_wgrad_group(gs, xs, self.dw, self.cs, flops=fl, V=self.saved_v, dU=du, fuse_dgrad_input=FUSE_DY, side=side,
                                            flags=flags, lists=lists)
            self.saved_v = None
            return
# ... 411 lines not shown
                s, names = L.spec, L.grad_names()
                cout, cin, kh, kw = L.weight.shape
                j = _hip.UnpackJob()
                j.dw, j.w_packed, j.dweight = L.dw.data_ptr(), L.wf.data_ptr(), views[names[0]].data_ptr()
                j.Cout, j.Cin, j.kh, j.kw, j.kw_pad, j.c_pad, j.Kpad = cout, cin, kh, kw, L.kw_pad, L.cin_pad, L.wf.shape[1]
                j.scale, j.mean, j.rstd, j.colsum = _hip.ptr(L.scale), _hip.ptr(L.mean), _hip.ptr(L.rstd), L.cs.data_ptr()
                j.dgamma = views[names[1]].data_ptr() if s.bn else None
                j.dbeta = views[names[-1]].data_ptr() if len(names) > 1 else None
                chunks.extend((len(jobs), co) for co in range(cout))
                jobs.append(j)
            arr = (_hip.UnpackJob * len(jobs))(*jobs)
            dev = layers[0].dw.device
            hit = cache[index] = (key, torch.frombuffer(bytearray(bytes(arr)), dtype=torch.uint8).to(dev),
                                  torch.tensor(chunks, dtype=torch.int32).to(dev), len(chunks))
        _hip.check(_hip.load().rn_unpack_batched(hit[1].data_ptr(), hit[2].data_ptr(), hit[3], _hip.stream()), "rn_unpack_batched")
        for L in layers:
            L.dw = L.cs = L.wd = L.uf = L.ud = L.saved_v = L.dy_v = None

    def _zero_grad_accumulators(self, device, flag_bytes=0, flag_arrays=0):
        wino = self.use_wino and not self.bwd16
        sizes = []
        for L in self.layers.values():
            s = L.spec
            du = 36 * s.cout * ((s.cin + 31) // 32 * 32) if (wino and L.wino_layer) else 0
            sizes.append((L, L.wf.numel(), (s.cout + 3) // 4 * 4, du))
        total = (sum(a + b + c for _, a, b, c in sizes) + 3) // 4 * 4
        acc_floats = total
        total += flag_arrays * flag_bytes // 4
        arena = getattr(self, "_arena", None)
        if arena is None or arena.numel() != total or arena.device != device:
            arena = self._arena = torch.empty(total, dtype=torch.float32, device=device)
        arena.zero_()
        o = 0
        for L, a, b, c in sizes:
            L.dw = arena[o:o + a].view_as(L.wf)
            L.cs = arena[o + a:o + a + L.spec.cout]
            L.du = arena[o + a + b:o + a + b + c].view(36, L.spec.cout, -1) if c else None
            o += a + b + c
        fb = arena[acc_floats:].view(torch.uint8)
        self._reg_flags = [fb[i * flag_bytes:(i + 1) * flag_bytes] for i in range(flag_arrays)]
        n = cv.tile_lists_numel(flag_bytes) if flag_arrays else 0
        bufs = getattr(self, "_reg_list_bufs", None)
        if flag_arrays and (bufs is None or len(bufs) != flag_arrays or bufs[0].numel() != n or bufs[0].device != device):
            bufs = self._reg_list_bufs = [torch.empty(n, dtype=torch.int32, device=device) for _ in range(flag_arrays)]
        self._reg_lists = bufs if flag_arrays else []

    def calibrate(self, P, frames, margin=1.0):
        if self.fp8 or self.bf16:
            raise RuntimeError("calibrate with the fp32 engine (ResNet.calibrate_fp8 switches to it): the magnitudes are recorded "
                               "by the fp32 direct kernels' path only")
        rec = {}
        wino_eval, self.wino_eval = self.wino_eval, False
        for L in self.layers.values():
            L.calib = rec
        self.calib = rec
        try:
            with torch.no_grad():
                self.forward(P, frames, save=False)
        finally:
            for L in self.layers.values():
                L.calib = None
            self.calib = None
            self.wino_eval = wino_eval
        missing = [n for n in self.fp8_scale_names() if n not in rec]
        assert not missing, "calibration pass did not record %s" % missing
        return {k: v * margin for k, v in rec.items()}

    def fp8_scale_names(self):
        return ["pool"] + [n for n in self.layers if n != "conv1" and not n.endswith(".output")]

    def set_fp8_layers(self, fp8=None, other="fp32"):
        assert self.fp8 and other in ("fp32", "bf16")
        pick = (lambda n: True) if fp8 is None else (fp8 if callable(fp8) else (lambda n, names=set(fp8): n in names))
        self._fp8_explicit = True
        on = []
        for n, L in self.layers.items():
            if n == "conv1":
                continue
            L.fwd_mode = "fp8" if pick(n) else other
            if L.fwd_mode == "fp8":
                on.append(n)
        return on

    def forward(self, P, img, save, x4=None):
        Ls = self.layers
        if save and os.environ.get("RN_BATCHED_PREP", "1") != "0":
            self._prepare_training(P)
        else:
            self._prepare(P)
        if self.fp8:
            if save and not self.fp8_trainable:
                raise RuntimeError("the fp8 training step (fp8 forward, bf16 gradients) is built for the bottleneck networks "
                                   "(resnet50/101/152), like the bf16 schedule")
            if not self.fp8_scales:
                raise RuntimeError("the fp8 engine needs activation scales: net.calibrate_fp8(frames) first")
            missing = [n_ for n_ in self.fp8_scale_names() if not self.fp8_scales.get(n_, 0.0) > 0.0]
            if missing:
                raise RuntimeError("fp8 activation scales are missing (or zero) for %d tensors, e.g. %s: run net.calibrate_fp8(frames) "
                                   "on representative frames" % (len(missing), ", ".join(missing[:4])))
            if getattr(self, "_fp8_explicit", None) is None:
                stream = (lambda n_: n_.endswith(".conv3") or ".downsample." in n_ or n_.startswith("fpn.") or n_ == "regressionModel.conv4") \
                    if self.fp8_policy == "stream_bf16" else (lambda n_: False)
                for n_, L in Ls.items():
                    if n_ != "conv1":
                        L.fwd_mode = "bf16" if stream(n_) else "fp8"
            if save and any(L.mode() == "fp32" for n_, L in Ls.items() if n_ != "conv1"):
                raise RuntimeError("the fp8 training step saves e4m3 / bf16 activations for the bf16 gradient kernels: no fp32-format layers")
            for n_, L in Ls.items():
                L.out_scale = max(self.fp8_scales.get(n_, 0.0), 1e-30) / cv.FP8_MAX
            pyr = ("fpn.P3_2", "fpn.P4_2", "fpn.P5_2", "fpn.P6", "fpn.P7_2")
            common = max(Ls[n_].out_scale for n_ in pyr)
            for n_ in pyr:
                Ls[n_].out_scale = common
        for L in Ls.values():
            L.wino_active = bool((save or self.wino_eval) and self.use_wino and L.wino_layer and not self.bf16 and not self.fp8)
            L.keep_v = bool(save)
            L.sign = bool(save) and not L.fp8 and (not L.bf16 or cv.BITMASKS_BF16)
        if x4 is None:
            _hip.need_gpu(img)
            x4 = cv.nchw_to_nhwc4(img)
        else:
            _hip.need_gpu(x4)
        B, H, W, _ = x4.shape
        S = {} if save else None
        stem = Ls["conv1"].fwd(x4, act=cv.ACT_RELU)
        pool = cv.maxpool_fwd_bf16 if self.bf16 else cv.maxpool_fwd
        if self.fp8 and not save and getattr(self, "calib", None) is None:
            x = cv.maxpool_fwd_fp8(stem, max(self.fp8_scales.get("pool", 0.0), 1e-30) / cv.FP8_MAX)
        else:
            if save:
                x, pool_arg = pool(stem, want_argmax=True)
                S["x4"], S["stem"], S["pool_arg"] = x4, stem, pool_arg
            else:
                x = pool(stem)
            if getattr(self, "calib", None) is not None:
                self.calib["pool"] = max(self.calib.get("pool", 0.0), float(x.abs().max()))
            if self.fp8:
                x = cv.fp8_quantize(x, max(self.fp8_scales.get("pool", 0.0), 1e-30) / cv.FP8_MAX)
        if save:
            S["blocks"] = []
        feats = {}
        for pre, roles in self.blocks:
            xin = x
            t1 = roles["conv1"].fwd(xin, act=cv.ACT_RELU)
            res = roles["down"].fwd(xin) if "down" in roles else xin
            if self.kind == "basic":
                t2 = None
                x = roles["conv2"].fwd(t1, act=cv.ACT_RELU, add=res, add_mode=1)
            else:
                t2 = roles["conv2"].fwd(t1, act=cv.ACT_RELU)
                x = roles["conv3"].fwd(t2, act=cv.ACT_RELU, add=res, add_mode=1)
            if save:
                S["blocks"].append((xin, t1, t2, x))
            feats[pre.split(".")[0]] = x
        c3, c4, c5 = feats["layer2"], feats["layer3"], feats["layer4"]
        p5lat = Ls["fpn.P5_1"].fwd(c5)
        p5 = Ls["fpn.P5_2"].fwd(p5lat)
        p4sum = Ls["fpn.P4_1"].fwd(c4, add=p5lat, add_mode=2, add_hw=(p5lat.shape[1], p5lat.shape[2]))
        p4 = Ls["fpn.P4_2"].fwd(p4sum)
        p3sum = Ls["fpn.P3_1"].fwd(c3, add=p4sum, add_mode=2, add_hw=(p4sum.shape[1], p4sum.shape[2]))
        p3 = Ls["fpn.P3_2"].fwd(p3sum)
        p6 = Ls["fpn.P6"].fwd(c5, sign=True)
        p6r = cv.relu_bf16(p6) if self.bf16 else None
        if self.fp8:
            p6r = torch.relu(_as_f32(p6))
            p6r._rn_qscale = _qscale(p6)
        p7 = Ls["fpn.P7_2"].fwd(p6r) if (self.bf16 or self.fp8) else Ls["fpn.P7_2"].fwd(p6, in_relu=True)
        pyramid = [p3, p4, p5, p6, p7]
        if save:
            S["fpn"] = (c3, c4, c5, p5lat, p4sum, p3sum, p6)
            S["p6r"] = p6r
            S["pyramid"] = pyramid
        counts = [f.shape[1] * f.shape[2] * arch.NUM_ANCHORS for f in pyramid]
        A = sum(counts)
        reg = torch.empty((B, A, self.n_reg), dtype=torch.float32, device=x4.device)
        cls = torch.empty((B, A, self.num_classes), dtype=torch.float32, device=x4.device)
        if save:
            S["towers"] = {"regressionModel": [], "classificationModel": []}
            S["counts"] = counts
        side = self.tower_streams(x4.device)
        main = torch.cuda.current_stream(x4.device)
        v_ready = None
        if side is not None:
            fork = main.record_event()
        for ti, (prefix, out, width, act) in enumerate((("regressionModel", reg, self.n_reg, cv.ACT_NONE),
                                                        ("classificationModel", cls, self.num_classes, cv.ACT_SIGMOID))):
            if side is not None:
                side[ti].wait_event(fork)
                if ti == 1 and v_ready is not None:
                    side[ti].wait_event(v_ready)
            with torch.cuda.stream(side[ti] if side is not None else main):
                ts = pyramid
                acts = []
                for i in range(1, 5):
                    first = Ls["regressionModel.conv1"]
                    shared = first.saved_v if (i == 1 and prefix == "classificationModel") else None
                    ts = Ls["%s.conv%d" % (prefix, i)].fwd_group(ts, act=cv.ACT_RELU, wino=save and self.use_wino and not self.bf16 and not self.fp8,
                                                                 shared_v=shared)
                    acts.append(ts)
                    if side is not None and ti == 0 and i == 1:
                        v_ready = side[0].record_event()
                views, off = [], 0
                for cnt in counts:
                    views.append(out.view(B, -1)[:, off * width:])
                    off += cnt
                Ls[prefix + ".output"].fwd_group(ts, act=act, outs=views, y_batch_stride=A * width)
            if save:
                S["towers"][prefix] = [[acts[i][li] for i in range(4)] for li in range(5)]
        if side is not None:
            main.wait_stream(side[0])
            main.wait_stream(side[1])
        if save:
            S["wino_v"] = {n: L.saved_v for n, L in Ls.items() if L.saved_v is not None}
        for L in Ls.values():
            L.saved_v = None
        return reg, cls, S

    def backward(self, S, dreg, dcls, cls):
        Ls = self.layers
        grads = {}
        sparse_reg = SPARSE_REG and self.use_wino and not self.bwd16 and not self.bf16 and not self.fp8 and dreg.is_cuda
        reg_tiles = [dreg.shape[0] * ((f.shape[1] + 3) // 4) * ((f.shape[2] + 3) // 4) for f in S["pyramid"]]
        self._zero_grad_accumulators(dreg.device, cv.wino_tpad(sum(reg_tiles)) if sparse_reg else 0, 5 if sparse_reg else 0)
        for L in Ls.values():
            L.saved_v = L.dy_v = None
        for n, v in S.pop("wino_v", {}).items():
            Ls[n].saved_v = v

        flat = views = None
        next_bucket = 0
        if self.flat_bucket_bytes:
            flat, views = self._flat_views(dreg.device)
            buckets = self._flat["buckets"]

        batched = flat is not None and self.grad_hook is None and os.environ.get("RN_BATCHED_UNPACK", "1") != "0"
        pending = []

        main0 = torch.cuda.current_stream(dreg.device) if dreg.is_cuda else None
        wss = self.wgrad_streams(dreg.device) if batched else None
        wg_count = 0
        held = []

        def join():
            for ws in wss or ():
                main0.wait_stream(ws)
                cv.side_release(ws)
            held.clear()

        def aside(fn, tensors):
            nonlocal wg_count
            ws = wss[wg_count % len(wss)]
            wg_count += 1
            if cv.want_amax():
                for t in tensors:
                    if t.dtype == torch.float32 and t.is_contiguous():
                        cv.amax_words(t)
            ws.wait_event(torch.cuda.current_stream(dreg.device).record_event())
            with torch.cuda.stream(ws):
                fn()
            held.append(tuple(tensors) + tuple(getattr(t, "_rn_amax", (None,))[0] for t in tensors))

        def wg(L, g, x, in_relu=False):
            if wss is None:
                L.bwd_params(g, x, in_relu=in_relu)
            elif L.wino_active and not L.bf16:
                L.bwd_params(g, x, in_relu=in_relu, side=wss[0] if os.environ.get("RN_WGRAD_WINO", "1") != "0" else None)
            else:
                aside(lambda: L.bwd_params(g, x, in_relu=in_relu), (g, x))

        def wg_group(L, gs, xs, wino=False, flags=None, lists=None):
            if wss is None or os.environ.get("RN_WGRAD_TOWERS", "0") == "0":
                L.bwd_params_group(gs, xs, wino=wino, flags=flags, lists=lists)
            elif wino or L.wino_active:
                L.bwd_params_group(gs, xs, wino=wino, side=wss[0], flags=flags, lists=lists)
            else:
                aside(lambda: L.bwd_params_group(gs, xs), tuple(gs) + tuple(xs))

        def fused(L, g, x):
            return cv.BWD_FUSED_1X1 and not self.bwd16 and not self.fp8 and self.grad_hook is None and L.bwd_fused_ok(g, x)

        def done(layer):
            nonlocal next_bucket
            if batched:
                pending.append(layer)
                grads.update({n: views[n] for n in layer.grad_names()})
            else:
                g = layer.finish(views)
                grads.update(g)
                if self.grad_hook is not None:
# ... 157 lines not shown
```

### 3d-playground_amd/retinanet_mi355x/modules.py

```python
import math

import torch
import torch.nn as nn

from . import _hip, arch, engine, ops, torch_ops


class BasicBlock(nn.Module):
    expansion = 1

    def __init__(self, inplanes, planes, stride=1, downsample=None):
        super().__init__()
        self.conv1 = nn.Conv2d(inplanes, planes, 3, stride, 1, bias=False)
        self.bn1 = nn.BatchNorm2d(planes)
        self.relu = nn.ReLU(inplace=True)
        self.conv2 = nn.Conv2d(planes, planes, 3, 1, 1, bias=False)
        self.bn2 = nn.BatchNorm2d(planes)
        self.downsample = downsample
        self.stride = stride


class Bottleneck(nn.Module):
    expansion = 4

# ... 28 lines not shown

class _Tower(nn.Module):
    def __init__(self, num_features_in, n_out, feature_size):
        super().__init__()
        for i in range(1, 5):
            setattr(self, "conv%d" % i, nn.Conv2d(num_features_in if i == 1 else feature_size, feature_size, 3, padding=1))
            setattr(self, "act%d" % i, nn.ReLU())
        self.output = nn.Conv2d(feature_size, n_out, 3, padding=1)


class RegressionModel(_Tower):
    def __init__(self, num_features_in, num_anchors=9, feature_size=256, n_outputs=8):
        super().__init__(num_features_in, num_anchors * n_outputs, feature_size)
        self.n_outputs = n_outputs


class ClassificationModel(_Tower):
    def __init__(self, num_features_in, num_anchors=9, num_classes=80, prior=0.01, feature_size=256):
        super().__init__(num_features_in, num_anchors * num_classes, feature_size)
        self.num_classes = num_classes
        self.num_anchors = num_anchors
        self.output_act = nn.Sigmoid()


class Anchors(nn.Module):
    def __init__(self, pyramid_levels=None, strides=None, sizes=None, ratios=None, scales=None):
        super().__init__()
        if not (pyramid_levels is None and strides is None and sizes is None and ratios is None and scales is None):
            raise NotImplementedError("the reference ignores every non-default argument except by crashing "
                                      "(D/anchors.py:9-19 only assigns the attributes in the None branches)")
        self.pyramid_levels = [3, 4, 5, 6, 7]
        self.strides = [2 ** x for x in self.pyramid_levels]
        self.sizes = [2 ** (x + 2) for x in self.pyramid_levels]

    def forward(self, image):
        if not image.is_cuda:
            raise RuntimeError("anchors are generated on the MI355X (no CPU fallback); got device %s" % image.device)
        return torch.ops.retinanet_mi355x.anchors(image.shape[2], image.shape[3], image.device)


class BBoxTransform(nn.Module):
    def __init__(self, mean=None, std=None, directional=True):
        super().__init__()
        if mean is not None or std is not None:
            raise NotImplementedError("custom mean/std: the directional transform never reads them (D/utils.py:102-149) "
                                      "and every caller of the 2D one uses the defaults (R/model.py:196)")
        self.directional = directional

    def forward(self, boxes, regression):
        if self.directional:
            return torch.ops.retinanet_mi355x.decode_dir(boxes, regression)
        return torch.ops.retinanet_mi355x.decode_2d(boxes, regression, False, 0, 0)


class ClipBoxes(nn.Module):
    def __init__(self, width=None, height=None):
        super().__init__()

    def forward(self, boxes, img):
        ops.clip_boxes_check(boxes)
        torch.ops.retinanet_mi355x.clip_boxes_(boxes, img.shape[2], img.shape[3])
        return boxes


class FocalLoss(nn.Module):
    def __init__(self, directional=True):
        super().__init__()
        self.directional = directional

    def forward(self, classifications, regressions, anchors, annotations):
        return torch_ops.focal_loss(classifications, regressions, anchors, annotations, self.directional)


def calc_iou(a, b):
    return torch.ops.retinanet_mi355x.pairwise_iou(a, b)


class _NetFn(torch.autograd.Function):

    @staticmethod
    def forward(ctx, net, img, ann, *params):
        eng = net._engine
        P = net._tensor_dict()
        reg, cls, S = eng.forward(P, img, save=True)
        anc = eng.anchors(img.shape[2], img.shape[3], img.device)
        lib = _hip.load()
        ann_c = _hip.f32c(ann)
        B, A, C = cls.shape
        ws = ops.focal_workspace(B, A, img.device)
        losses = torch.empty(3, dtype=torch.float32, device=img.device)
        _hip.check(lib.rn_focal_loss_fwd(cls.data_ptr(), reg.data_ptr(), anc.data_ptr(), _hip.ptr(ann_c), B, A, C,
                                         ann_c.shape[1], int(net.directional), ws.data_ptr(), losses.data_ptr(),
                                         _hip.stream()), "rn_focal_loss_fwd")
        ctx.net, ctx.S, ctx.pack = net, S, (reg, cls, anc, ann_c, ws)
        return losses[0:1], losses[1:2], losses[2:3]

    @staticmethod
    def backward(ctx, g_cls, g_reg, g_vp):
        net, S = ctx.net, ctx.S
        reg, cls, anc, ann_c, ws = ctx.pack
        ctx.S = ctx.pack = None
        lib = _hip.load()
        B, A, C = cls.shape
        g = torch.cat([t.reshape(1).float() for t in (g_cls, g_reg, g_vp)])
        dcls, dreg = torch.empty_like(cls), torch.empty_like(reg)
        _hip.check(lib.rn_focal_loss_bwd(cls.data_ptr(), reg.data_ptr(), anc.data_ptr(), _hip.ptr(ann_c), B, A, C,
                                         ann_c.shape[1], int(net.directional), ws.data_ptr(), g.data_ptr(),
                                         dcls.data_ptr(), dreg.data_ptr(), _hip.stream()), "rn_focal_loss_bwd")
        red = net.__dict__.get("_reducer")
        eng = net._engine
        if red is not None:
            red.backward_begins()
        grads = eng.backward(S, dreg, dcls, cls)
        if red is not None:
            red.finalize_flat(eng._flat["arena"])
        return (None, None, None) + tuple(grads[n] for n in eng.param_names)


class ResNet(nn.Module):

    def __init__(self, num_classes, block, layers, directional=True):
        self.inplanes = 64
        super().__init__()
        self.directional = directional
        self.ingest_swap_rb = False
        self.ingest_mean, self.ingest_std = ops.IMAGENET_MEAN, ops.IMAGENET_STD
        self.conv1 = nn.Conv2d(3, 64, kernel_size=7, stride=2, padding=3, bias=False)
        self.bn1 = nn.BatchNorm2d(64)
        self.relu = nn.ReLU(inplace=True)
        self.maxpool = nn.MaxPool2d(kernel_size=3, stride=2, padding=1)
        self.layer1 = self._make_layer(block, 64, layers[0])
        self.layer2 = self._make_layer(block, 128, layers[1], stride=2)
        self.layer3 = self._make_layer(block, 256, layers[2], stride=2)
        self.layer4 = self._make_layer(block, 512, layers[3], stride=2)
        e = block.expansion
        self.fpn = PyramidFeatures(128 * e, 256 * e, 512 * e)
        n_reg = 12 if directional else 4
        self.regressionModel = RegressionModel(256, n_outputs=n_reg)
        self.classificationModel = ClassificationModel(256, num_classes=num_classes)
        self.anchors = Anchors()
        self.regressBoxes = BBoxTransform(directional=directional)
        self.clipBoxes = ClipBoxes()
        self.focalLoss = FocalLoss(directional=directional)
        for m in self.modules():
            if isinstance(m, nn.Conv2d):
                n = m.kernel_size[0] * m.kernel_size[1] * m.out_channels
                m.weight.data.normal_(0, math.sqrt(2. / n))
            elif isinstance(m, nn.BatchNorm2d):
                m.weight.data.fill_(1)
                m.bias.data.zero_()
        prior = 0.01
        self.classificationModel.output.weight.data.fill_(0)
        self.classificationModel.output.bias.data.fill_(-math.log((1.0 - prior) / prior))
        self.regressionModel.output.weight.data.fill_(0)
        self.regressionModel.output.bias.data.fill_(0)
        self.freeze_bn()
        arch_name = {(BasicBlock, (2, 2, 2, 2)): "resnet18", (BasicBlock, (3, 4, 6, 3)): "resnet34",
                     (Bottleneck, (3, 4, 6, 3)): "resnet50", (Bottleneck, (3, 4, 23, 3)): "resnet101",
                     (Bottleneck, (3, 8, 36, 3)): "resnet152"}.get((block, tuple(layers)))
        if arch_name is None:
            raise ValueError("Block type %s / layers %s not understood" % (block, layers))
        self.__dict__["_arch_name"] = arch_name
        self.__dict__["_engine"] = engine.Engine(arch_name, num_classes, n_reg)

    def _make_layer(self, block, planes, blocks, stride=1):
        downsample = None
        if stride != 1 or self.inplanes != planes * block.expansion:
            downsample = nn.Sequential(
                nn.Conv2d(self.inplanes, planes * block.expansion, kernel_size=1, stride=stride, bias=False),
                nn.BatchNorm2d(planes * block.expansion))
# ... 120 lines not shown
```

### include/retinanet_mi355x.h

```cpp
#ifndef RETINANET_MI355X_H
#define RETINANET_MI355X_H

#include <stdint.h>

#ifdef __cplusplus
extern "C" {
#endif

#define RN_OK 0
#define RN_EINVAL 10001
#define RN_ETOOMANY 10002
#define RN_MAX_GT 256
#define RN_LEVELS 5

const char *rn_version(void);
int rn_check_device(void);

int64_t rn_anchor_count(int height, int width);
void rn_anchor_base_boxes(double out[RN_LEVELS * 9 * 4]);
int rn_anchors_fwd(float *out, int height, int width, void *stream);

int rn_pairwise_iou(const float *a, const float *b, float *iou, int64_t A, int N, void *stream);

int64_t rn_focal_workspace_bytes(int B, int64_t A);
int64_t rn_focal_workspace_zero_bytes(int B);
int rn_focal_loss_fwd(const float *cls, const float *reg, const float *anchors, const float *ann,
                      int B, int64_t A, int C, int N, int directional,
                      void *workspace, float *losses, void *stream);
int rn_focal_loss_bwd(const float *cls, const float *reg, const float *anchors, const float *ann,
                      int B, int64_t A, int C, int N, int directional,
                      const void *workspace, const float *grad_losses,
                      float *dcls, float *dreg, void *stream);
int rn_assign(const float *anchors, const float *ann, int B, int64_t A, int N, int directional,
              float *iou_max, int32_t *argmax, int32_t *state, void *stream);

int rn_decode_dir(const float *anchors, const float *reg, float *boxes, int B, int64_t A, void *stream);
int rn_decode_dir_select(const float *anchors, const float *reg, int64_t A, const float *scores, int64_t score_stride,
                         const int32_t *sel_idx, const int32_t *count, int max_candidates, float *boxes,
                         float *cand_scores, int32_t *cand_image, void *stream);
int rn_decode_2d(const float *anchors, const float *deltas, float *boxes, int B, int64_t A,
                 int clip, float width, float height, void *stream);
int rn_clip_boxes(float *boxes, int64_t n, float width, float height, void *stream);

int64_t rn_post_workspace_bytes(int64_t n_scores, int64_t max_candidates);
int rn_rowmax(const float *cls, int64_t n, int C, float *scores, int64_t *classes, void *stream);
int rn_threshold_select(const float *scores, int64_t n, int64_t stride, double start, int keep,
                        double fixed_threshold, void *workspace, int32_t *count, int32_t *sel_idx, void *stream);
int rn_nms(const float *boxes, int64_t box_stride, int box_col, const float *scores, int64_t score_stride,
           const int32_t *cand_idx, const int32_t *category, const int32_t *count, int max_candidates,
           float iou_thr, void *workspace, int32_t *keep, int32_t *keep_count, void *stream);

int rn_state_to_space(const float *state, float *space, int64_t d, void *stream);
int rn_space_to_state(const double *space, float *state, int64_t d, void *stream);
int rn_state_to_im(const float *state, const double *P, const double *P2, const int32_t *mat_index,
                   double *im, int64_t d, void *stream);
int rn_space_to_im(const float *space, const double *P, const double *P2, const int32_t *mat_index,
                   double *im, int64_t d, void *stream);
int rn_im_to_space(const double *im, const float *heights, const double *H, const double *H2,
                   const int32_t *mat_index, double *space, int64_t d, void *stream);
int rn_im_to_state(const double *im, const float *heights, const double *H, const double *H2,
                   const int32_t *mat_index, float *state, int64_t d, void *stream);

#define RN_PARSE_MAX 16384
int64_t rn_parse_workspace_bytes(int64_t d);
int rn_parse_detections(const float *scores, const int64_t *labels, const float *boxes20, const int64_t *camera_idxs,
                        int64_t d, const double *H1, const double *H2, const double *P1, const double *P2, int n_cam,
                        const float *heights, float sigma_d, float phi_nms_im, float phi_nms_space,
                        int perform_nms, int refine_height, void *workspace,
                        float *out_state, int64_t *out_labels, float *out_scores, int64_t *out_cams,
                        int32_t *out_count, void *stream);
int rn_md_iou(const double *a, const double *b, double *out, int64_t n, void *stream);

int rn_crop_boxes(const double *im_objs, const int64_t *cam_idxs, int n, double b, double *crop_boxes, float *rois,
                  void *stream);
int rn_roi_align(const float *frames, int N, int C, int H, int W, const float *rois, int n, int out_h, int out_w,
                 float *out, int nhwc4, void *stream);
int rn_crop_select(const float *reg_boxes, const float *cls, const double *crop_boxes, const int64_t *cam_idxs,
                   const float *pre_loc, const double *H1, const double *H2, const double *P1, const double *P2,
                   int n_cam, int n, int A, int C, double cs, int cd_max, float W, float *out_state, int64_t *out_cls,
                   float *out_conf, void *stream);

int rn_kf_view(const float *X, const float *D, const float *F, const double *dt, int dt_is_tensor, int with_direction,
               float *out, int n, void *stream);
int rn_kf_predict(float *X, float *P, const float *D, double *T, const float *F, const float *Q, const double *dt,
                  int dt_is_tensor, double dt_default, int n, void *stream);
int rn_kf_update(float *X, float *P, const int32_t *rows, const double *z, const float *H, const float *R,
                 const float *mu_R, int m, void *stream);

#define RN_LSAP_MAX_MIN 4096
int rn_track_cost(const float *pre, int64_t pre_stride, const float *det, int64_t det_stride, int64_t n, int64_t m,
                  double *cost, void *stream);
int64_t rn_lsap_workspace_bytes(int64_t nr, int64_t nc);
int rn_linear_sum_assignment(const double *cost, int64_t nr, int64_t nc, double max_cost, void *workspace,
                             int32_t *row_match, int32_t *n_matched, int32_t *status, void *stream);

#define RN_TS_MAX_CAMS 1024
int64_t rn_ts_bias_workspace_bytes(int64_t d, int64_t max_pairs);
int rn_estimate_ts_bias(const float *boxes, int64_t box_stride, const int64_t *camera_idxs, int64_t d,
                        const int32_t *d_count, const float *objs, int64_t obj_stride, int64_t n,
                        const double *timestamps, double *ts_bias, int n_cam, double phi, double alpha, float mu_v,
                        void *workspace, int64_t max_pairs, int32_t *pairs_out, float *te_out, int32_t *info,
                        void *stream);

int rn_track_crop_prior(const float *X, const float *D, const double *T, const float *F, const float *centers,
                        const double *stamps, const double *bias, int n_cam, float *pre_loc, int32_t *cam, double *dt,
                        int n, void *stream);

#define RN_FIT_MAX (1 << 24)
#define RN_MOMENTS_MAX_K 8
#define RN_MOMENTS_MAX_G 16
int rn_fit_nearest(const float *gt, const float *det, const int32_t *offsets, int64_t B, int64_t D, int32_t *rows,
                   float *resid, int32_t *info, void *stream);
int rn_residual_moments(const float *E, int64_t N, int k, const int32_t *group, int G, float *mean, float *cov,
                        int32_t *count, void *stream);

#define RN_EVAL_MAX_K (1 << 20)
#define RN_EVAL_MAX_DET 4096
// ... 166 lines not shown
                  int Cin, int Ho, int Wo, int Cout, int kh, int kw, int stride, int pad, int in_relu, void *stream);
int rn_conv_wgrad_batched(const float *dy, int ldy, const float *x, float *dw, float *colsum, int nbatch,
                          int64_t dy_bstride, int64_t x_bstride, int64_t dw_bstride, int colsum_batch, int N, int Hi, int Wi,
                          int Cin, int Ho, int Wo, int Cout, int kh, int kw, int stride, int pad, int in_relu,
                          const void *dy_amax, int dy_amax_n, const void *x_amax, int x_amax_n, void *stream);
int64_t rn_conv_wgrad_det_workspace_bytes(int ldy, int nbatch, int64_t dw_bstride, int N, int Hi, int Wi, int Cin, int Ho, int Wo,
                                          int Cout, int kh, int kw);
int rn_conv_wgrad_batched_det(const float *dy, int ldy, const float *x, float *dw, float *colsum, int nbatch,
                              int64_t dy_bstride, int64_t x_bstride, int64_t dw_bstride, int colsum_batch, int N, int Hi, int Wi,
                              int Cin, int Ho, int Wo, int Cout, int kh, int kw, int stride, int pad, int in_relu,
                              const void *dy_amax, int dy_amax_n, const void *x_amax, int x_amax_n, void *workspace, int64_t workspace_bytes,
                              void *stream);
int rn_conv_wgrad_batched_flags(const float *dy, int ldy, const float *x, float *dw, float *colsum, int nbatch,
                                int64_t dy_bstride, int64_t x_bstride, int64_t dw_bstride, int colsum_batch, int N, int Hi, int Wi,
                                int Cin, int Ho, int Wo, int Cout, int kh, int kw, int stride, int pad, int in_relu,
                                const void *dy_amax, int dy_amax_n, const void *x_amax, int x_amax_n, const void *k_active,
                                void *workspace, int64_t workspace_bytes, void *stream);
int rn_conv_wgrad_plan(int ldy, int nbatch, int64_t dy_bstride, int64_t x_bstride, int64_t dw_bstride, int colsum_batch, int N, int Hi,
                       int Wi, int Cin, int Ho, int Wo, int Cout, int kh, int kw, int stride, int pad, int in_relu, int have_amax,
                       int have_flags, int det, int32_t *out);
int rn_conv_bwd_1x1(const float *dy, const float *x, const void *w_split, const float *w_unscale, float *dx, float *dw, float *colsum,
                    const void *mask, int mask_mode, const float *add, void *sign_out, const void *dy_amax, const void *x_amax,
                    void *dx_amax, int N, int H, int W, int Cin, int Cout, int stride, void *stream);

int rn_f32_to_bf16(const float *src, void *dst, int64_t n, void *stream);
int rn_bf16_to_f32(const void *src, float *dst, int64_t n, void *stream);
int rn_conv_igemm_bf16(const rn_conv_desc *d, const void *x, const void *w_packed, void *y, int y_is_f32,
                       const float *scale, const float *shift, const void *add, const void *mask, void *stream);
int rn_conv_igemm_bf16_grouped(const rn_conv_group *g, const void *w_packed, int y_is_f32, const float *scale,
                               const float *shift, void *stream);
int rn_conv_igemm_bf16_tile_rows(const rn_conv_group *g, int y_is_f32);
int rn_fp8_quantize(const float *src, void *dst, int64_t n, float inv_scale, void *stream);
int rn_maxpool_fwd_fp8out(const float *x, void *y, int N, int H, int W, int C, int Ho, int Wo, float inv_scale, void *stream);
int rn_fp8_dequantize(const void *src, float *dst, int64_t n, float scale, void *stream);
int rn_fp8_to_bf16(const void *src, void *dst, int64_t n, float scale, void *stream);
int rn_bf16_to_fp8(const void *src, void *dst, int64_t n, float inv_scale, void *stream);
int rn_fp8_quantize_rows(const float *w_packed, void *w_q, float *row_scale, int64_t rows, int Kpad, void *stream);
int rn_conv_igemm_fp8(const rn_conv_desc *d, const void *x_q, const void *w_q, void *y, int y_is_f32, const float *scale,
                      const float *shift, const void *add_q, float add_scale, float out_inv_scale, void *stream);
int rn_conv_igemm_fp8_tile_rows(const rn_conv_group *g, int y_is_f32);
int rn_conv_igemm_fp8_tile(const rn_conv_desc *d, int y_is_f32);
int rn_conv_igemm_bf16_tile(const rn_conv_desc *d, int y_is_f32);
int rn_conv_igemm_fp8_grouped(const rn_conv_group *g, const void *w_q, int y_is_f32, const float *scale, const float *shift,
                              float add_scale, float out_inv_scale, void *stream);

int rn_conv_wgrad_bf16(const void *dy, int ldy, const void *x, float *dw, float *colsum, int N, int Hi, int Wi, int Cin,
                       int Ho, int Wo, int Cout, int kh, int kw, int stride, int pad, void *stream);
int rn_conv_wgrad_bf16_grouped(int n, const void *const *dy, int ldy, const void *const *x, float *dw, float *colsum, int N,
                               const int *Hi, const int *Wi, int Cin, int Cout, int kh, int kw, int stride, int pad, void *stream);

int rn_maxpool_fwd_bf16out(const float *x, void *y, uint8_t *argmax, int N, int H, int W, int C, int Ho, int Wo, void *stream);
int rn_maxpool_bwd_bf16in(const float *x, const void *dy, const uint8_t *argmax, float *dx, int N, int H, int W, int C, int Ho,
                          int Wo, int relu_mask, void *stream);
int rn_upsample_add_bwd_bf16(const void *src, void *dst, int N, int Hs, int Ws, int Hd, int Wd, int C, void *stream);
int rn_sigmoid_bwd_pad_bf16(const float *dy, const float *s, void *out, int B, int64_t rows_per_image, int C, int ld,
                            int64_t src_batch_stride, void *stream);
int rn_relu_bf16(const void *src, void *dst, int64_t n, void *stream);

typedef struct rn_wino_group {
    int n;
    int N[RN_MAX_GROUP], H[RN_MAX_GROUP], W[RN_MAX_GROUP];
    const float *src[RN_MAX_GROUP];
    float *dst[RN_MAX_GROUP];
    const float *add[RN_MAX_GROUP];
    const float *mask[RN_MAX_GROUP];
    void *sign[RN_MAX_GROUP];
    void *amax[RN_MAX_GROUP];
} rn_wino_group;
int rn_wino_input_group(const rn_wino_group *g, float *V, int C, int64_t tile_offset, int64_t Tpad, int dy_form,
                        void *row_amax, void *tensor_amax, void *stream);
int rn_wino_input_both_group(const rn_wino_group *g, float *V, float *Z, int C, int64_t tile_offset, int64_t Tpad,
                             void *v_row_amax, void *z_tensor_amax, void *stream);
int rn_wino_output_group(const rn_wino_group *g, const float *M, int Cout, int64_t tile_offset, int64_t Tpad,
                         const float *scale, const float *shift, int mask_mode, int act, int64_t y_batch_stride, void *stream);
int rn_wino_input_both_group_flags(const rn_wino_group *g, float *V, float *Z, int C, int64_t tile_offset, int64_t Tpad,
                                   void *v_row_amax, void *z_tensor_amax, const void *flags, void *stream);
int rn_wino_output_group_flags(const rn_wino_group *g, const float *M, int Cout, int64_t tile_offset, int64_t Tpad,
                               const float *scale, const float *shift, int mask_mode, int act, int64_t y_batch_stride,
                               const void *flags_in, void *flags_out, void *stream);
int rn_tile_lists(const void *flags, int64_t Tpad, void *counts, void *tiles, void *units, void *blocks, void *stream);
int rn_wino_input_both_group_lists(const rn_wino_group *g, float *V, float *Z, int C, int64_t tile_offset, int64_t Tpad,
                                   void *v_row_amax, void *z_tensor_amax, const void *flags, const void *units, const void *n_units,
                                   void *stream);
int rn_wino_input(const float *x, float *V, int N, int H, int W, int C, int64_t tile_offset, int64_t Tpad, void *stream);
int rn_wino_output(const float *M, float *y, int N, int H, int W, int Cout, int64_t tile_offset, int64_t Tpad,
                   const float *scale, const float *shift, const float *add, const float *mask, int mask_mode, int act,
                   int64_t y_batch_stride, void *stream);
int rn_wino_weights(const float *w, float *U, int Cout, int Cin, int mode, const float *scale, void *stream);
int rn_wino_dy(const float *dy, float *Z, int N, int H, int W, int C, int64_t tile_offset, int64_t Tpad, void *stream);
int rn_wino_dw(const float *dU, float *dw, int Cout, int Cin, void *stream);

typedef struct rn_prep_job {
    int kind;
    int Cout, Cin, kh, kw, kw_pad, c_pad, mode, r0, nr, s0, ns, rows, Kpad;
    float eps;
    const float *src;
    float *dst;
    const float *scale;
    const float *gamma, *beta, *mean, *var;
    float *bn_scale, *bn_shift, *bn_rstd;
} rn_prep_job;
int rn_prep_batched(const rn_prep_job *jobs_dev, const int32_t *chunks_dev, int nchunks, void *stream);

int rn_pack_weights(const float *src, float *dst, int Cout, int Cin, int kh, int kw, int kw_pad, int c_pad,
                    int mode, const float *scale, int r0, int nr, int s0, int ns, void *stream);
int rn_unpack_wgrad(const float *dw, const float *w_packed, float *dweight, int Cout, int Cin, int kh, int kw,
                    int kw_pad, int c_pad, const float *scale, const float *mean, const float *rstd,
                    const float *colsum, float *dgamma, float *dbeta, void *stream);

typedef struct rn_unpack_job {
    const float *dw, *w_packed;
    float *dweight;
    int Cout, Cin, kh, kw, kw_pad, c_pad, Kpad;
    const float *scale, *mean, *rstd, *colsum;
    float *dgamma, *dbeta;
} rn_unpack_job;
int rn_unpack_batched(const rn_unpack_job *jobs_dev, const int32_t *chunks_dev, int nchunks, void *stream);

int rn_bn_fold(const float *gamma, const float *beta, const float *mean, const float *var, float eps, int C,
               float *scale, float *shift, float *rstd, void *stream);

int rn_nchw_to_nhwc4(const float *src, float *dst, int N, int H, int W, void *amax, void *stream);
int rn_maxpool_fwd(const float *x, float *y, uint8_t *argmax, int N, int H, int W, int C, int Ho, int Wo, void *stream);
int rn_maxpool_bwd(const float *x, const float *dy, const uint8_t *argmax, float *dx, int N, int H, int W, int C,
                   int Ho, int Wo, int relu_mask, void *amax, void *stream);
int rn_colsum(const float *g, int64_t rows, int C, int ld, float *out, int accumulate, void *workspace, void *stream);
int64_t rn_colsum_workspace_bytes(int64_t rows, int C);
int rn_upsample_add_bwd(const float *src, float *dst, int N, int Hs, int Ws, int Hd, int Wd, int C, void *amax, void *stream);
int rn_relu_mask(float *g, const float *z, int64_t n, void *stream);
int rn_sigmoid_bwd_pad(const float *dy, const float *s, float *out, int B, int64_t rows_per_image, int C, int ld,
                       int64_t src_batch_stride, void *amax, void *stream);
int rn_sigmoid_bwd_pad_flags(const float *dy, const float *s, float *out, int B, int H, int W, int C, int ld,
                             int64_t src_batch_stride, void *amax, void *flags, void *stream);
int rn_add_inplace(float *dst, const float *src, int64_t n, int64_t per_image, void *amax, void *stream);

int64_t rn_opt_workspace_bytes(int n_chunks);
int rn_opt_clip_adam(const void *tensor_table, const void *chunk_table, int n_chunks, float max_norm, float lr,
                     float beta1, float beta2, float eps, int step, int write_clipped, void *workspace,
                     float *total_norm, void *stream);
int rn_opt_clip_adam_dev(const void *tensor_table, const void *chunk_table, int n_chunks, float max_norm, float lr,
                         float beta1, float beta2, float eps, int *step_dev, int write_clipped, void *workspace,
                         float *total_norm, void *stream);
int rn_opt_clip_adam_hp(const void *tensor_table, const void *chunk_table, int n_chunks, const float *hp, int *step_dev,
                        int write_clipped, void *workspace, float *total_norm, void *stream);

#define RN_MOT_MAX 512
#define RN_MOT_MAX_IDS 16384
#define RN_MOT_RESULT 152
#define RN_MOT_OK 0
#define RN_MOT_INVALID 1
#define RN_MOT_INFEASIBLE 2
#define RN_MOT_TOO_LARGE 3
int rn_mot_prepare(const double *gt_im, const float *gt_h0, const float *gt_vel, int64_t G, const float *pred_state,
                   int64_t M, const double *H, const double *P, float *gt_state, float *gt_box, float *pred_box,
                   double *pred_im, void *stream);
int rn_mot_iou(const float *gt_box, const float *pred_box, const int32_t *gt_off, const int32_t *pr_off,
               const int64_t *iou_off, int64_t F, int64_t max_cells, double *iou, void *stream);
int rn_mot_assign(const double *iou, const int32_t *gt_off, const int32_t *pr_off, const int64_t *iou_off,
                  const int32_t *slot_off, int64_t F, int64_t max_n, int64_t S, int64_t M, int32_t *slot_row,
                  int32_t *slot_col, uint8_t *pred_assigned, int32_t *frame_status, void *stream);
int rn_mot_frame_metrics(const double *iou, const int32_t *gt_off, const int32_t *pr_off, const int64_t *iou_off,
                         const int32_t *slot_off, int64_t F, int64_t S, const int32_t *slot_row, const int32_t *slot_col,
                         const int32_t *frame_status, double match_iou, const float *gt_state, const float *pred_state,
                         const double *gt_im, const double *pred_im, const int32_t *gt_cls, const int32_t *pred_cls,
                         const int32_t *gt_id, const int32_t *pred_id, const uint8_t *pred_assigned, double *slot_iou,
                         int32_t *slot_gid, int32_t *slot_pid, float *slot_state_err, double *slot_bot, double *slot_top,
// ... 253 lines not shown
```

Baseline: 137.7 images/sec.

## Compute regression tower forward only on Winograd tiles near positive anchors

A new kernel marks the Winograd output tiles that hold anchors with IoU of at least 0.5 against the ground-truth boxes. It then dilates that set layer by layer to cover the receptive field of the four-conv regression tower. New list-driven Winograd input and output kernels transform and write only those tiles, and fill the rest with zeros. The aim is to skip regression-head forward work whose outputs never reach the regression loss. The cost is extra anchor matching and dilation passes before the forward. The path is disabled once CUDA-graph capture has been seen and under reduced precision, and regression outputs outside the needed tiles are no longer valid.

After: 144.3 images/sec, median of 6. 1.05x the previous value.

```diff
diff --git a/3d-playground_amd/csrc/conv_wino.hip b/3d-playground_amd/csrc/conv_wino.hip
--- a/3d-playground_amd/csrc/conv_wino.hip
+++ b/3d-playground_amd/csrc/conv_wino.hip
@@ -122,15 +122,89 @@
     }
 }
 
-template <bool PBITS, bool PADD, bool FLAGS = false>
+__global__ __launch_bounds__(256) void wino_in_list_kernel(const WinoTable g, float *__restrict__ V, int C, int64_t t0, int64_t Tpad,
+                                                           unsigned *__restrict__ row_amax, unsigned *__restrict__ tensor_amax,
+                                                           const unsigned char *__restrict__ flags, const int *__restrict__ units,
+                                                           const int *__restrict__ n_units) {
+    wino_tensor_word(g, tensor_amax, WINO_GAIN_BT);
+    const int cq = C >> 2;
+    const int64_t id = (int64_t)blockIdx.x * 256 + threadIdx.x;
+    const int64_t t_last = g.tile_end[g.n - 1];
+    const int64_t it = id / cq;
+    const int c4 = (int)(id - it * cq) * 4;
+    const int nu_raw = *n_units, nu_max = (int)(Tpad >> 4);
+    const int64_t rows = 16 * (int64_t)(nu_raw < 0 ? 0 : (nu_raw < nu_max ? nu_raw : nu_max));
+    if ((id - threadIdx.x) >= rows * cq) return;
+    int64_t gt_raw = it < rows ? (int64_t)units[it >> 4] * 16 + (it & 15) - t0 : t_last;
+    if (gt_raw < 0) gt_raw = t_last;
+    const int64_t gt = gt_raw < t_last ? gt_raw : t_last - 1;
+    int64_t tile;
+    const int q = wino_locate(g, gt, tile);
+    const float *x = g.src[0];
+    const unsigned *xw = g.amax[0];
+    WINO_SELECT(q, g, pr, x = g.src[i_]; xw = g.amax[i_];)
+    const int H = pr.H, W = pr.W, TW = pr.TW;
+    const int n = (int)(tile / (pr.TH * TW));
+    const int r = (int)(tile - (int64_t)n * pr.TH * TW);
+    const int th = r / TW, tw = r - th * TW;
+    const int h0 = 4 * th - 1, w0 = 4 * tw - 1;
+    const float *xb = x + (int64_t)n * H * W * C + c4;
+    const bool needed = gt_raw < t_last && flags[t0 + gt] != 0;
+    if (row_amax != nullptr) {
+        const int e_img = rn_amax_exp_lanes(xw != nullptr ? reinterpret_cast<const unsigned char *>(xw) + (int64_t)n * RN_AMAX_BYTES : nullptr);
+        if (needed && c4 == 0) row_amax[t0 + gt] = rn_amax_word_of_exp(e_img, WINO_GAIN_BT);
+    }
+    if (gt_raw >= t_last) return;
+    float *vb = V + (t0 + gt) * C + c4;
+    if (!needed) {
+#pragma unroll
+        for (int p = 0; p < 36; ++p) st_stream(vb + (int64_t)p * Tpad * C, f4(0.f));
+        return;
+    }
+    float4 t[6][6];
+#pragma unroll
+    for (int j = 0; j < 6; ++j) {
+        float4 d[6], o[6];
+        const int w = w0 + j;
+#pragma unroll
+        for (int i = 0; i < 6; ++i) {
+            const int h = h0 + i;
+            const bool ok = (unsigned)h < (unsigned)H && (unsigned)w < (unsigned)W;
+            d[i] = ok ? *reinterpret_cast<const float4 *>(xb + ((int64_t)h * W + w) * C) : f4(0.f);
+        }
+        bt6(d, o);
+#pragma unroll
+        for (int i = 0; i < 6; ++i) t[i][j] = o[i];
+    }
+#pragma unroll
+    for (int i = 0; i < 6; ++i) {
+        float4 o[6];
+        bt6(t[i], o);
+#pragma unroll
+        for (int j = 0; j < 6; ++j) st_stream(vb + (int64_t)(i * 6 + j) * Tpad * C, o[j]);
+    }
+}
+
+template <bool PBITS, bool PADD, bool FLAGS = false, bool LIST = false>
 __global__ __launch_bounds__(256, 2) void wino_out_kernel(const WinoTable g, const float *__restrict__ M, int Cout, int64_t t0,
                                                        int64_t Tpad, const float *__restrict__ scale,
                                                        const float *__restrict__ shift, int mask_mode, int act, int64_t y_bs,
                                                        const unsigned char *__restrict__ fin = nullptr,
-                                                       unsigned char *__restrict__ fout = nullptr) {
+                                                       unsigned char *__restrict__ fout = nullptr,
+                                                       const int *__restrict__ tiles = nullptr,
+                                                       const int *__restrict__ n_tiles = nullptr) {
     const int cq = Cout >> 2;
     const int64_t id = (int64_t)blockIdx.x * 256 + threadIdx.x;
-    const int64_t gt = id / cq;
+    const int64_t it = id / cq;
+    int64_t gt_sel = it;
+    if constexpr (LIST) {
+        const int nt_raw = *n_tiles;
+        const int64_t nt = nt_raw < 0 ? 0 : (nt_raw < Tpad ? nt_raw : Tpad);
+        if ((id - threadIdx.x) / cq >= nt) return;
+        gt_sel = it < nt ? (int64_t)tiles[it] - t0 : g.tile_end[g.n - 1];
+        if (gt_sel < 0) gt_sel = g.tile_end[g.n - 1];
+    }
+    const int64_t gt = gt_sel;
     float am = 0.f;
     unsigned *yam = nullptr;
     int n_img = 0;
@@ -138,7 +212,7 @@
     do {
     if (gt >= g.tile_end[g.n - 1]) break;
     live = true;
-    const int c4 = (int)(id - gt * cq) * 4;
+    const int c4 = (int)(id - it * cq) * 4;
     int64_t tile;
     const int q = wino_locate(g, gt, tile);
     float *y = g.dst[0];
@@ -597,6 +671,24 @@
     return RN_OK;
 }
 
+extern "C" int rn_wino_input_group_list(const rn_wino_group *g, float *V, int C, int64_t tile_offset, int64_t Tpad, void *row_amax,
+                                        void *tensor_amax, const void *flags, const void *units, const void *n_units, void *stream) {
+    WinoTable t;
+    const int rc = wino_table(g, t);
+    if (rc) return rc;
+    if (!V || C <= 0 || (C & 3) || tile_offset < 0 || tile_offset + t.tile_end[t.n - 1] > Tpad) return RN_EINVAL;
+    if (!flags || !units || !n_units || ((uintptr_t)units & 3) || ((uintptr_t)n_units & 3) || (Tpad & 15)) return RN_EINVAL;
+    for (int i = 0; i < t.n; ++i)
+        if (!t.src[i]) return RN_EINVAL;
+    const dim3 gl(rn_blocks(Tpad * (C >> 2), 256));
+    hipLaunchKernelGGL(wino_in_list_kernel, gl, dim3(256), 0, (hipStream_t)stream, t, V, C, tile_offset, Tpad,
+                       reinterpret_cast<unsigned *>(row_amax), reinterpret_cast<unsigned *>(tensor_amax),
+                       reinterpret_cast<const unsigned char *>(flags), reinterpret_cast<const int *>(units),
+                       reinterpret_cast<const int *>(n_units));
+    RN_LAUNCH_CHECK();
+    return RN_OK;
+}
+
 extern "C" int rn_wino_input_both_group(const rn_wino_group *g, float *V, float *Z, int C, int64_t tile_offset, int64_t Tpad,
                                         void *v_row_amax, void *z_tensor_amax, void *stream) {
     return rn_wino_input_both_group_flags(g, V, Z, C, tile_offset, Tpad, v_row_amax, z_tensor_amax, nullptr, stream);
@@ -642,6 +734,36 @@
                                     void *stream) {
     return rn_wino_output_group_flags(g, M, Cout, tile_offset, Tpad, scale, shift, mask_mode, act, y_batch_stride, nullptr, nullptr, stream);
 }
+extern "C" int rn_wino_output_group_list(const rn_wino_group *g, const float *M, int Cout, int64_t tile_offset, int64_t Tpad,
+                                         const float *scale, const float *shift, int mask_mode, int act, int64_t y_batch_stride,
+                                         const void *tiles, const void *n_tiles, void *stream) {
+    WinoTable t;
+    const int rc = wino_table(g, t);
+    if (rc) return rc;
+    if (Cout <= 0 || (Cout & 3) || tile_offset < 0 || tile_offset + t.tile_end[t.n - 1] > Tpad) return RN_EINVAL;
+    if (!tiles || !n_tiles || ((uintptr_t)tiles & 3) || ((uintptr_t)n_tiles & 3)) return RN_EINVAL;
+    if (mask_mode < 0 || (mask_mode & ~(3 | RN_MASK_BITS)) || (mask_mode & 3) == 3 || mask_mode == RN_MASK_BITS) return RN_EINVAL;
+    if (act < 0 || act > 2 || y_batch_stride < 0 || (y_batch_stride & 3)) return RN_EINVAL;
+    for (int i = 0; i < t.n; ++i) {
+        if (!t.dst[i] || (mask_mode != 0) != (t.mask[i] != nullptr)) return RN_EINVAL;
+        if (((mask_mode & RN_MASK_BITS) || t.sign[i]) && (Cout & 31)) return RN_EINVAL;
+        if (y_batch_stride && y_batch_stride < (int64_t)t.p[i].H * t.p[i].W * Cout) return RN_EINVAL;
+    }
+    const bool pbits = (mask_mode & RN_MASK_BITS) != 0;
+    bool padd = true;
+    for (int i = 0; i < t.n; ++i) padd = padd && t.add[i] != nullptr;
+    const dim3 grid(rn_blocks(Tpad * (Cout >> 2), 256));
+#define RN_WINO_OUT_L(B, A) hipLaunchKernelGGL((wino_out_kernel<B, A, false, true>), grid, dim3(256), 0, (hipStream_t)stream, t, M, Cout, tile_offset, \
+                                               Tpad, scale, shift, mask_mode, act, y_batch_stride, (const unsigned char *)nullptr,                   \
+                                               (unsigned char *)nullptr, reinterpret_cast<const int *>(tiles), reinterpret_cast<const int *>(n_tiles))
+    if (pbits && padd) RN_WINO_OUT_L(true, true);
+    else if (pbits) RN_WINO_OUT_L(true, false);
+    else if (padd) RN_WINO_OUT_L(false, true);
+    else RN_WINO_OUT_L(false, false);
+#undef RN_WINO_OUT_L
+    RN_LAUNCH_CHECK();
+    return RN_OK;
+}
 
 static rn_wino_group wino_single(const float *src, float *dst, const float *add, const float *mask, int N, int H, int W) {
     rn_wino_group g = {};
diff --git a/3d-playground_amd/csrc/focal_loss.hip b/3d-playground_amd/csrc/focal_loss.hip
--- a/3d-playground_amd/csrc/focal_loss.hip
+++ b/3d-playground_amd/csrc/focal_loss.hip
@@ -840,6 +840,103 @@
     return RN_OK;
 }
 
+struct NeedGeom {
+    int n;
+    int W[RN_MAX_GROUP], TH[RN_MAX_GROUP], TW[RN_MAX_GROUP];
+    int64_t a_end[RN_MAX_GROUP];
+    int64_t t_end[RN_MAX_GROUP];
+};
+
+template <bool DIR>
+__global__ __launch_bounds__(NTHR) void need_p0_kernel(const float4 *__restrict__ anchors, const float *__restrict__ ann, int64_t A, int N,
+                                                       int per_pixel, const NeedGeom g, unsigned char *__restrict__ p0) {
+    constexpr int COLS = DIR ? 27 : 5;
+    __shared__ LabelLds L;
+    const int j = blockIdx.y;
+    load_labels<DIR>(ann + (int64_t)j * N * COLS, N, L);
+    const int64_t ai = (int64_t)blockIdx.x * NTHR + threadIdx.x;
+    if (ai >= A || L.count == 0) return;
+    float best; int arg;
+    match_anchor(anchors[ai], L, best, arg);
+    if (!(best >= 0.5f)) return;
+    int q = 0;
+#pragma unroll
+    for (int i = 0; i < RN_MAX_GROUP - 1; ++i) q += (i + 1 < g.n && ai >= g.a_end[i]) ? 1 : 0;
+    const int64_t a_first = q ? g.a_end[q - 1] : 0, t_first = q ? g.t_end[q - 1] : 0;
+    const int64_t pix = (ai - a_first) / per_pixel;
+    const int h = (int)(pix / g.W[q]), w = (int)(pix - (int64_t)h * g.W[q]);
+    p0[t_first + ((int64_t)j * g.TH[q] + (h >> 2)) * g.TW[q] + (w >> 2)] = 1;
+}
+
+__global__ __launch_bounds__(256) void need_dilate_kernel(const NeedGeom g, int64_t T, int64_t Tpad, unsigned char *__restrict__ flags) {
+    const int64_t t = (int64_t)blockIdx.x * 256 + threadIdx.x;
+    if (t >= T) return;
+    int q = 0;
+#pragma unroll
+    for (int i = 0; i < RN_MAX_GROUP - 1; ++i) q += (i + 1 < g.n && t >= g.t_end[i]) ? 1 : 0;
+    const int64_t t_first = q ? g.t_end[q - 1] : 0;
+    const int TH = g.TH[q], TW = g.TW[q];
+    const int64_t local = t - t_first;
+    const int64_t n = local / ((int64_t)TH * TW);
+    const int r = (int)(local - n * TH * TW);
+    const int th = r / TW, tw = r - th * TW;
+    const unsigned char *img = flags + t_first + n * TH * TW;
+    int dmin = 6;
+    for (int dh = -5; dh <= 5; ++dh) {
+        const int th2 = th + dh;
+        if ((unsigned)th2 >= (unsigned)TH) continue;
+        for (int dw = -5; dw <= 5; ++dw) {
+            const int tw2 = tw + dw;
+            if ((unsigned)tw2 >= (unsigned)TW) continue;
+            if (img[th2 * TW + tw2] != 0) {
+                const int a = dh < 0 ? -dh : dh, b = dw < 0 ? -dw : dw, d = a > b ? a : b;
+                dmin = d < dmin ? d : dmin;
+            }
+        }
+    }
+#pragma unroll
+    for (int k = 1; k <= 4; ++k)
+        if (dmin <= k + 1) flags[k * Tpad + t] = 1;
+    if (dmin <= 1) flags[5 * Tpad + t] = 1;
+}
+
+__global__ __launch_bounds__(256) void need_zero_kernel(uint4 *__restrict__ p, int64_t n16) {
+    const int64_t i = (int64_t)blockIdx.x * 256 + threadIdx.x;
+    if (i < n16) p[i] = make_uint4(0u, 0u, 0u, 0u);
+}
+
+extern "C" int rn_reg_need_tiles(const float *anchors, const float *ann, int B, int64_t A, int N, int directional, int n_levels,
+                                 const int *H, const int *W, int per_pixel, void *flags, int64_t Tpad, void *stream) {
+    const int rc = check_args(B, A, 1, N);
+    if (rc) return rc;
+    if (!anchors || (N > 0 && !ann) || !H || !W || !flags || n_levels < 1 || n_levels > RN_MAX_GROUP || per_pixel < 1) return RN_EINVAL;
+    if (Tpad <= 0 || (Tpad & 15) || ((uintptr_t)flags & 15)) return RN_EINVAL;
+    NeedGeom g = {};
+    g.n = n_levels;
+    int64_t a = 0, t = 0;
+    for (int i = 0; i < RN_MAX_GROUP; ++i) {
+        const int k = i < n_levels ? i : n_levels - 1;
+        if (H[k] <= 0 || W[k] <= 0) return RN_EINVAL;
+        g.W[i] = W[k]; g.TH[i] = (H[k] + 3) / 4; g.TW[i] = (W[k] + 3) / 4;
+        if (i < n_levels) { a += (int64_t)H[k] * W[k] * per_pixel; t += (int64_t)B * g.TH[i] * g.TW[i]; }
+        g.a_end[i] = a; g.t_end[i] = t;
+    }
+    if (a != A || t > Tpad) return RN_EINVAL;
+    hipStream_t s = (hipStream_t)stream;
+    const int64_t n16 = (int64_t)RN_REG_NEED_ARRAYS * Tpad / 16;
+    hipLaunchKernelGGL(need_zero_kernel, dim3(rn_blocks(n16, 256)), dim3(256), 0, s, reinterpret_cast<uint4 *>(flags), n16);
+    RN_LAUNCH_CHECK();
+    const dim3 grid((unsigned)((A + NTHR - 1) / NTHR), B), block(NTHR);
+    const float4 *anc = reinterpret_cast<const float4 *>(anchors);
+    unsigned char *f = reinterpret_cast<unsigned char *>(flags);
+    if (directional) hipLaunchKernelGGL(need_p0_kernel<true>, grid, block, 0, s, anc, ann, A, N, per_pixel, g, f);
+    else hipLaunchKernelGGL(need_p0_kernel<false>, grid, block, 0, s, anc, ann, A, N, per_pixel, g, f);
+    RN_LAUNCH_CHECK();
+    hipLaunchKernelGGL(need_dilate_kernel, dim3(rn_blocks(t, 256)), dim3(256), 0, s, g, t, Tpad, f);
+    RN_LAUNCH_CHECK();
+    return RN_OK;
+}
+
 __global__ void pairwise_iou_kernel(const float4 *__restrict__ a, const float4 *__restrict__ b, float *__restrict__ out,
                                     int64_t A, int N) {
     const int64_t i = (int64_t)blockIdx.x * 256 + threadIdx.x;
diff --git a/3d-playground_amd/retinanet_mi355x/_hip.py b/3d-playground_amd/retinanet_mi355x/_hip.py
--- a/3d-playground_amd/retinanet_mi355x/_hip.py
+++ b/3d-playground_amd/retinanet_mi355x/_hip.py
@@ -30,6 +30,7 @@
     "rn_focal_loss_fwd": (c_i32, [c_vp, c_vp, c_vp, c_vp, c_i32, c_i64, c_i32, c_i32, c_i32, c_vp, c_vp, c_vp]),
     "rn_focal_loss_bwd": (c_i32, [c_vp, c_vp, c_vp, c_vp, c_i32, c_i64, c_i32, c_i32, c_i32, c_vp, c_vp, c_vp, c_vp, c_vp]),
     "rn_assign": (c_i32, [c_vp, c_vp, c_i32, c_i64, c_i32, c_i32, c_vp, c_vp, c_vp, c_vp]),
+    "rn_reg_need_tiles": (c_i32, [c_vp, c_vp, c_i32, c_i64, c_i32, c_i32, c_i32, c_vp, c_vp, c_i32, c_vp, c_i64, c_vp]),
     "rn_decode_dir": (c_i32, [c_vp, c_vp, c_vp, c_i32, c_i64, c_vp]),
     "rn_decode_dir_select": (c_i32, [c_vp, c_vp, c_i64, c_vp, c_i64, c_vp, c_vp, c_i32, c_vp, c_vp, c_vp, c_vp]),
     "rn_decode_2d": (c_i32, [c_vp, c_vp, c_vp, c_i32, c_i64, c_i32, c_f32, c_f32, c_vp]),
@@ -160,6 +161,7 @@
 
 
 RN_MAX_GROUP = 5
+RN_REG_NEED_ARRAYS = 6
 
 
 class ConvGroup(ctypes.Structure):
@@ -194,6 +196,8 @@
     "rn_wino_input_both_group": (c_i32, [ctypes.POINTER(WinoGroup), c_vp, c_vp, c_i32, c_i64, c_i64, c_vp, c_vp, c_vp]),
     "rn_wino_input_both_group_flags": (c_i32, [ctypes.POINTER(WinoGroup), c_vp, c_vp, c_i32, c_i64, c_i64, c_vp, c_vp, c_vp, c_vp]),
     "rn_tile_lists": (c_i32, [c_vp, c_i64, c_vp, c_vp, c_vp, c_vp, c_vp]),
+    "rn_wino_input_group_list": (c_i32, [ctypes.POINTER(WinoGroup), c_vp, c_i32, c_i64, c_i64, c_vp, c_vp, c_vp, c_vp, c_vp, c_vp]),
+    "rn_wino_output_group_list": (c_i32, [ctypes.POINTER(WinoGroup), c_vp, c_i32, c_i64, c_i64, c_vp, c_vp, c_i32, c_i32, c_i64, c_vp, c_vp, c_vp]),
     "rn_wino_input_both_group_lists": (c_i32, [ctypes.POINTER(WinoGroup), c_vp, c_vp, c_i32, c_i64, c_i64, c_vp, c_vp, c_vp, c_vp, c_vp, c_vp]),
     "rn_wino_output_group_flags": (c_i32, [ctypes.POINTER(WinoGroup), c_vp, c_i32, c_i64, c_i64, c_vp, c_vp, c_i32, c_i32, c_i64, c_vp, c_vp, c_vp]),
     "rn_wino_output_group": (c_i32, [ctypes.POINTER(WinoGroup), c_vp, c_i32, c_i64, c_i64, c_vp, c_vp, c_i32, c_i32, c_i64, c_vp]),
diff --git a/3d-playground_amd/retinanet_mi355x/conv.py b/3d-playground_amd/retinanet_mi355x/conv.py
--- a/3d-playground_amd/retinanet_mi355x/conv.py
+++ b/3d-playground_amd/retinanet_mi355x/conv.py
@@ -392,6 +392,60 @@
     return rows, tword
 
 
+NEED_POISON = False
+DENSE = "dense"
+
+
+def _need_fill(t, fill):
+    if NEED_POISON:
+        t.fill_(float("nan")) if t.is_floating_point() else t.fill_(-1)
+    elif fill == "zero":
+        t.zero_()
+    return t
+
+
+def _wino_transform_in_list(xs, V, C, Tpad, lists, want_tensor=False):
+    lib = _hip.load()
+    assert len(xs) <= _hip.RN_MAX_GROUP and lists.flags.numel() >= Tpad
+    am = want_amax()
+    rows = torch.zeros(Tpad, dtype=torch.int32, device=V.device) if am else None
+    tword = amax_single(V.device) if am and want_tensor else None
+    t = sum(x.shape[0] * ((x.shape[1] + 3) // 4) * ((x.shape[2] + 3) // 4) for x in xs)
+    g = _wino_group(xs, srcs=xs, amaxs=[amax_words(x) for x in xs] if am else None)
+    nb = 4.0 * (sum(x.numel() for x in xs) + 36 * t * C)
+    _hip.check(prof.timed("wino_input", nb, lambda: lib.rn_wino_input_group_list(
+        ctypes.byref(g), V.data_ptr(), C, 0, Tpad, _hip.ptr(rows), _hip.ptr(tword), lists.flags.data_ptr(), lists.units.data_ptr(),
+        lists.counts.data_ptr() + 4, _hip.stream())), "rn_wino_input_group_list")
+    return rows, tword
+
+
+class RegNeed:
+    __slots__ = ("flags", "lists", "hws", "B", "Tpad")
+
+
+def reg_need_tiles(anchors, ann, directional, B, hws, per_pixel, flag_buf=None, list_bufs=None):
+    lib = _hip.load()
+    dev = anchors.device
+    _hip.need_gpu(anchors, ann)
+    n = _hip.RN_REG_NEED_ARRAYS
+    T = sum(B * ((h + 3) // 4) * ((w + 3) // 4) for h, w in hws)
+    Tpad = wino_tpad(T)
+    A = anchors.numel() // 4
+    if flag_buf is None:
+        flag_buf = torch.empty(n * Tpad, dtype=torch.uint8, device=dev)
+    assert flag_buf.dtype == torch.uint8 and flag_buf.numel() == n * Tpad and anchors.is_contiguous() and ann.is_contiguous()
+    assert ann.dtype == torch.float32 and anchors.dtype == torch.float32 and ann.shape[0] == B
+    Hs = (ctypes.c_int * len(hws))(*[h for h, _ in hws])
+    Ws = (ctypes.c_int * len(hws))(*[w for _, w in hws])
+    _hip.check(lib.rn_reg_need_tiles(anchors.data_ptr(), _hip.ptr(ann) if ann.numel() else None, B, A, ann.shape[1], int(directional),
+                                     len(hws), Hs, Ws, per_pixel, flag_buf.data_ptr(), Tpad, _hip.stream()), "rn_reg_need_tiles")
+    r = RegNeed()
+    r.flags = [flag_buf[k * Tpad:(k + 1) * Tpad] for k in range(n)]
+    r.lists = [tile_lists(f, Tpad, buf=None if list_bufs is None else list_bufs[k]) for k, f in enumerate(r.flags)]
+    r.hws, r.B, r.Tpad = [tuple(x) for x in hws], B, Tpad
+    return r
+
+
 def _wino_workspace(device, floats_v, floats_m):
     key = (device, torch.cuda.current_stream(device).cuda_stream)
     ws = _WINO_WS.get(key)
@@ -440,11 +494,15 @@
 
 
 def wino_conv_group(xs, U, outs=None, scale=None, shift=None, act=ACT_NONE, adds=None, masks=None, mask_mode=2,
-                    flops=0.0, keep_v=False, y_batch_stride=0, V_in=None, V_ready=None, sign=False, flags_out=None):
+                    flops=0.0, keep_v=False, y_batch_stride=0, V_in=None, V_ready=None, sign=False, flags_out=None,
+                    need=None, need_in=None, need_fill=None):
     lib = _hip.load()
     dev = xs[0].device
     C = xs[0].shape[3]
     cout = U.shape[1]
+    if need is not None:
+        assert V_ready is None and flags_out is None and len(xs) <= _hip.RN_MAX_GROUP
+        need_in = need if need_in is None else need_in
     tiles = [x.shape[0] * ((x.shape[1] + 3) // 4) * ((x.shape[2] + 3) // 4) for x in xs]
     T = sum(tiles)
     Tpad = wino_tpad(T)
@@ -458,17 +516,29 @@
         V = V_in[0]
     elif keep_v:
         V = torch.empty(36 * Tpad * C, dtype=torch.float32, device=dev)
+        if need is not None and need_in is not DENSE:
+            _need_fill(V, need_fill)
+    if need is not None and NEED_POISON:
+        M[:36 * Tpad * cout].fill_(float("nan"))
+        if not keep_v and not reuse:
+            V[:36 * Tpad * C].fill_(float("nan"))
     assert all(x.is_contiguous() for x in xs)
     v_am = (None, None)
     if reuse:
         src = V_ready if ready else V_in
         v_am = src[2] if len(src) > 2 and src[2] is not None else (None, None)
+    elif need is not None and need_in is not DENSE:
+        assert need_in.flags.numel() >= Tpad
+        v_am = _wino_transform_in_list(xs, V, C, Tpad, need_in, want_tensor=keep_v)
     else:
         v_am = _wino_transform_in(xs, V, C, Tpad, 0, want_rows=True, want_tensor=keep_v)
     flags = V_ready[3] if ready and len(V_ready) > 3 else None
     lists = V_ready[4] if ready and len(V_ready) > 4 else None
     if flags_out is not None:
         assert flags_out.dtype == torch.uint8 and flags_out.numel() >= Tpad and len(xs) <= _hip.RN_MAX_GROUP
+    if need is not None:
+        assert need.flags.numel() >= Tpad
+        lists = need
     Vv = V[:36 * Tpad * C].view(36, 1, Tpad, C)
     Mv = M[:36 * Tpad * cout].view(36, 1, Tpad, cout)
     Uv = _carry_split(U, U.view(36 * cout, U.shape[2]))
@@ -478,6 +548,9 @@
                x_amax=v_am[0], x_amax_rows=True, row_active=flags, row_list=lists)
     if outs is None:
         outs = [torch.empty((x.shape[0], x.shape[1], x.shape[2], cout), dtype=torch.float32, device=dev) for x in xs]
+        if need is not None:
+            for o in outs:
+                _need_fill(o, need_fill)
     off = 0
     for k in range(0, len(xs), _hip.RN_MAX_GROUP):
         sl = slice(k, k + _hip.RN_MAX_GROUP)
@@ -494,7 +567,14 @@
         nops = 1 + (pa is not None and pa[0] is not None) + (1.0 / 32 if mbits else 1.0) * has_mask + (1.0 / 32 if signs[0] is not None else 0.0)
         nb = 4.0 * (36 * t * cout + nops * sum(x.shape[0] * x.shape[1] * x.shape[2] for x in part) * cout)
         mm = (mask_mode | (MASK_BITS if mbits else 0)) if has_mask else 0
-        if flags is not None or flags_out is not None:
+        if need is not None:
+            for w_ in signs:
+                if w_ is not None:
+                    _need_fill(w_, need_fill)
+            _hip.check(prof.timed("wino_output", nb, lambda: lib.rn_wino_output_group_list(
+                ctypes.byref(g), M.data_ptr(), cout, off, Tpad, _hip.ptr(scale), _hip.ptr(shift), mm,
+                act, y_batch_stride, need.tiles.data_ptr(), need.counts.data_ptr(), _hip.stream())), "rn_wino_output_group_list")
+        elif flags is not None or flags_out is not None:
             _hip.check(prof.timed("wino_output", nb, lambda: lib.rn_wino_output_group_flags(
                 ctypes.byref(g), M.data_ptr(), cout, off, Tpad, _hip.ptr(scale), _hip.ptr(shift), mm,
                 act, y_batch_stride, _hip.ptr(flags), _hip.ptr(flags_out), _hip.stream())), "rn_wino_output_group_flags")
diff --git a/3d-playground_amd/retinanet_mi355x/engine.py b/3d-playground_amd/retinanet_mi355x/engine.py
--- a/3d-playground_amd/retinanet_mi355x/engine.py
+++ b/3d-playground_amd/retinanet_mi355x/engine.py
@@ -8,6 +8,7 @@
 FUSE_DY = os.environ.get("RN_WINO_FUSE_DY", "1") != "0"
 SPARSE_REG = os.environ.get("RN_SPARSE_REG", "1") != "0"
 SPARSE_REG_LISTS = os.environ.get("RN_SPARSE_REG_LISTS", "1") != "0"
+SPARSE_REG_FWD = os.environ.get("RN_SPARSE_REG_FWD", "1") != "0"
 GROUPED_WGRAD_BF16 = os.environ.get("RN_GROUPED_WGRAD_BF16", "1") != "0"
 S2_SHORTCUT_COMPACT = os.environ.get("RN_S2_SHORTCUT_COMPACT", "1") != "0"
 STEM_BF16_PRODUCTS = os.environ.get("RN_STEM_BF16_PRODUCTS", "1") != "0"
@@ -201,7 +202,8 @@
                                  add=add, add_mode=add_mode, add_hw=add_hw, act=act, y_batch_stride=y_batch_stride,
                                  out_scale=self.out_scale, flops=self.flops(x.shape[0], Ho, Wo))
 
-    def fwd_group(self, xs, act=cv.ACT_NONE, outs=None, y_batch_stride=None, wino=False, shared_v=None):
+    def fwd_group(self, xs, act=cv.ACT_NONE, outs=None, y_batch_stride=None, wino=False, shared_v=None, need=None, need_in=None,
+                  need_fill=None):
         s = self.spec
         mode = self.mode()
         if self.fp8:
@@ -241,9 +243,10 @@
             fl = sum(self.flops(x.shape[0], x.shape[1], x.shape[2]) for x in xs)
             r = cv.wino_conv_group(xs, self.wino_weights(0), outs=outs, scale=self.scale, shift=self.shift, act=act, flops=fl,
                                    keep_v=self.keep_v, y_batch_stride=y_batch_stride or 0, V_in=shared_v if self.keep_v else None,
-                                   sign=self.sign and act == cv.ACT_RELU)
+                                   sign=self.sign and act == cv.ACT_RELU, need=need, need_in=need_in, need_fill=need_fill)
             ys, self.saved_v = r if self.keep_v else (r, None)
             return ys
+        assert need is None, "%s does not take the Winograd form: no need sets" % s.name
         probs, ys, fl = [], [], 0.0
         for i, x in enumerate(xs):
             N, Hi, Wi, _ = x.shape
@@ -821,7 +824,29 @@
                 on.append(n)
         return on
 
-    def forward(self, P, img, save, x4=None):
+    def reg_need(self, anchors, ann, directional, B, H, W):
+        if not (SPARSE_REG_FWD and self.use_wino and not self.bwd16 and not self.bf16 and not self.fp8 and ann.is_cuda):
+            return None
+        if torch.cuda.is_current_stream_capturing():
+            self._captured_once = True
+        if getattr(self, "_captured_once", False):
+            return None
+        Lout, L4 = self.layers["regressionModel.output"], self.layers["regressionModel.conv4"]
+        hws = arch.pyramid_shapes(H, W)
+        T = sum(B * ((h + 3) // 4) * ((w + 3) // 4) for h, w in hws)
+        if not (Lout.wino_layer and L4.wino_layer and cv.wino_flags_ok(T, L4.spec.cin, L4.spec.cout)
+                and cv.wino_flags_ok(T, Lout.spec.cin, Lout.spec.cout) and len(hws) <= _hip.RN_MAX_GROUP):
+            return None
+        Tpad, n = cv.wino_tpad(T), _hip.RN_REG_NEED_ARRAYS
+        fb = getattr(self, "_reg_need_flag_buf", None)
+        if fb is None or fb.numel() != n * Tpad or fb.device != ann.device:
+            fb = self._reg_need_flag_buf = torch.empty(n * Tpad, dtype=torch.uint8, device=ann.device)
+            self._reg_need_list_bufs = [torch.empty(cv.tile_lists_numel(Tpad), dtype=torch.int32, device=ann.device) for _ in range(n)]
+        need = cv.reg_need_tiles(anchors, ann, directional, B, hws, arch.NUM_ANCHORS, flag_buf=fb, list_bufs=self._reg_need_list_bufs)
+        self._reg_need_flags, self._reg_need_lists = need.flags, need.lists
+        return need
+
+    def forward(self, P, img, save, x4=None, reg_need=None):
         Ls = self.layers
         if save and os.environ.get("RN_BATCHED_PREP", "1") != "0":
             self._prepare_training(P)
@@ -920,6 +945,11 @@
         side = self.tower_streams(x4.device)
         main = torch.cuda.current_stream(x4.device)
         v_ready = None
+        need = reg_need if (save and reg_need is not None and reg_need.B == B and self.use_wino and not self.bf16 and not self.fp8
+                            and reg_need.hws == [(f.shape[1], f.shape[2]) for f in pyramid]) else None
+        need_fill = None if (SPARSE_REG and FUSE_DY) else "zero"
+        if need is not None and cv.NEED_POISON:
+            reg.fill_(float("nan"))
         if side is not None:
             fork = main.record_event()
         for ti, (prefix, out, width, act) in enumerate((("regressionModel", reg, self.n_reg, cv.ACT_NONE),
@@ -934,8 +964,10 @@
                 for i in range(1, 5):
                     first = Ls["regressionModel.conv1"]
                     shared = first.saved_v if (i == 1 and prefix == "classificationModel") else None
+                    nd = need.lists[5 - i] if (need is not None and ti == 0) else None
                     ts = Ls["%s.conv%d" % (prefix, i)].fwd_group(ts, act=cv.ACT_RELU, wino=save and self.use_wino and not self.bf16 and not self.fp8,
-                                                                 shared_v=shared)
+                                                                 shared_v=shared, need=nd, need_in=cv.DENSE if (nd is not None and i == 1) else None,
+                                                                 need_fill=need_fill if nd is not None else None)
                     acts.append(ts)
                     if side is not None and ti == 0 and i == 1:
                         v_ready = side[0].record_event()
@@ -943,7 +975,9 @@
                 for cnt in counts:
                     views.append(out.view(B, -1)[:, off * width:])
                     off += cnt
-                Ls[prefix + ".output"].fwd_group(ts, act=act, outs=views, y_batch_stride=A * width)
+                nd = need.lists[0] if (need is not None and ti == 0) else None
+                Ls[prefix + ".output"].fwd_group(ts, act=act, outs=views, y_batch_stride=A * width, need=nd,
+                                                 need_in=need.lists[5] if nd is not None else None, need_fill=need_fill if nd is not None else None)
             if save:
                 S["towers"][prefix] = [[acts[i][li] for i in range(4)] for li in range(5)]
         if side is not None:
diff --git a/3d-playground_amd/retinanet_mi355x/modules.py b/3d-playground_amd/retinanet_mi355x/modules.py
--- a/3d-playground_amd/retinanet_mi355x/modules.py
+++ b/3d-playground_amd/retinanet_mi355x/modules.py
@@ -134,10 +134,11 @@
     def forward(ctx, net, img, ann, *params):
         eng = net._engine
         P = net._tensor_dict()
-        reg, cls, S = eng.forward(P, img, save=True)
         anc = eng.anchors(img.shape[2], img.shape[3], img.device)
         lib = _hip.load()
         ann_c = _hip.f32c(ann)
+        need = eng.reg_need(anc, ann_c, net.directional, img.shape[0], img.shape[2], img.shape[3])
+        reg, cls, S = eng.forward(P, img, save=True, reg_need=need)
         B, A, C = cls.shape
         ws = ops.focal_workspace(B, A, img.device)
         losses = torch.empty(3, dtype=torch.float32, device=img.device)
diff --git a/include/retinanet_mi355x.h b/include/retinanet_mi355x.h
--- a/include/retinanet_mi355x.h
+++ b/include/retinanet_mi355x.h
@@ -33,6 +33,10 @@
                       float *dcls, float *dreg, void *stream);
 int rn_assign(const float *anchors, const float *ann, int B, int64_t A, int N, int directional,
               float *iou_max, int32_t *argmax, int32_t *state, void *stream);
+
+#define RN_REG_NEED_ARRAYS 6
+int rn_reg_need_tiles(const float *anchors, const float *ann, int B, int64_t A, int N, int directional, int n_levels,
+                      const int *H, const int *W, int per_pixel, void *flags, int64_t Tpad, void *stream);
 
 int rn_decode_dir(const float *anchors, const float *reg, float *boxes, int B, int64_t A, void *stream);
 int rn_decode_dir_select(const float *anchors, const float *reg, int64_t A, const float *scores, int64_t score_stride,
@@ -365,6 +369,11 @@
 int rn_wino_input_both_group_lists(const rn_wino_group *g, float *V, float *Z, int C, int64_t tile_offset, int64_t Tpad,
                                    void *v_row_amax, void *z_tensor_amax, const void *flags, const void *units, const void *n_units,
                                    void *stream);
+int rn_wino_input_group_list(const rn_wino_group *g, float *V, int C, int64_t tile_offset, int64_t Tpad, void *row_amax,
+                             void *tensor_amax, const void *flags, const void *units, const void *n_units, void *stream);
+int rn_wino_output_group_list(const rn_wino_group *g, const float *M, int Cout, int64_t tile_offset, int64_t Tpad,
+                              const float *scale, const float *shift, int mask_mode, int act, int64_t y_batch_stride,
+                              const void *tiles, const void *n_tiles, void *stream);
 int rn_wino_input(const float *x, float *V, int N, int H, int W, int C, int64_t tile_offset, int64_t Tpad, void *stream);
 int rn_wino_output(const float *M, float *y, int N, int H, int W, int Cout, int64_t tile_offset, int64_t Tpad,
                    const float *scale, const float *shift, const float *add, const float *mask, int mask_mode, int act,
```
